# CIS565-Fall-2017/Project3-CUDA-Path-Tracer

Hardware: AMD Instinct MI355X
Metric: Mrays/sec (live paths x bounces) at 800x800 Cornell depth 8 (higher is better)
Workload: dtype f32

## Files before the change

### include/ptmi355.h

```cpp
#ifndef PTMI355_H
#define PTMI355_H

#include <stdint.h>

#ifdef __cplusplus
extern "C" {
#endif

typedef struct pt_vec3 { float x, y, z; } pt_vec3;
typedef struct pt_mat4 { float m[4][4]; } pt_mat4;

enum pt_geom_type { PT_SPHERE = 0, PT_CUBE = 1,
                    PT_TRIANGLE_MESH = 2 };

typedef struct pt_ray { pt_vec3 origin, direction; } pt_ray;

typedef struct pt_geom {
    int32_t type;
    int32_t materialid;
    pt_vec3 translation, rotation, scale;
    pt_mat4 transform, inverseTransform, invTranspose;
} pt_geom;

typedef struct pt_material {
// ... 150 lines not shown
    float   normal_tolerance;
} pt_temporal_params;
int pt_denoise_temporal(const pt_denoise_params *params, const pt_temporal_params *temporal, int iter,
                        float *host_rgb, uint8_t *host_rgba);
int pt_history(float *rgb, float *length);
int pt_history_reset(void);

int pt_set_denoise_albedo(int enable);
int pt_albedo(float *rgb);

typedef struct pt_variance_params { int32_t levels; float sigma_luminance, sigma_normal, sigma_position; } pt_variance_params;
int pt_get_moments(float *m1, float *m2);
int pt_set_moments(const float *m1, const float *m2);
int pt_denoise_variance(const pt_variance_params *params, int iter, float *host_rgb, uint8_t *host_rgba);
int pt_variance(float *host_var);

int pt_denoise_svgf(const pt_variance_params *params, const pt_temporal_params *temporal, int spatial_below, int iter,
                    float *host_rgb, uint8_t *host_rgba);
int pt_svgf_history(float *rgb, float *u1, float *u2, float *length);
int pt_svgf_variance(float *host_var);
int pt_svgf_reset(void);
int pt_get_stats(pt_stats *stats);
long long pt_total_rays(void);
int pt_get_counters(int64_t *rays, int64_t *first_bounce_rays, int64_t *iterations);

enum pt_stage { PT_STAGE_RAYGEN = 0, PT_STAGE_BOUNCE = 1, PT_STAGE_INTERSECT = 2,
                PT_STAGE_SORT = 3, PT_STAGE_GATHER = 4, PT_STAGE_MESH = 5, PT_STAGE_COUNT = 6 };
typedef struct pt_profile {
    double  ms[PT_STAGE_COUNT];
    int64_t launches[PT_STAGE_COUNT];
} pt_profile;
int pt_set_profiling(int enable);
int pt_get_profile(pt_profile *out);
typedef struct pt_bvh_info {
    int32_t nodes, triangles, depth;
    float   pad;
    float   prune;
} pt_bvh_info;
int pt_get_bvh_info(pt_bvh_info *out);
int pt_bvh_build(const pt_triangle *triangles, int count, float *nodes, int node_capacity,
                 int32_t *order, float *grid);
int pt_cull_boxes(const pt_geom *geoms, int count, const float *eye, float *boxes, float *origin_bound, float *reject);
int pt_tri_bounds(const pt_triangle *triangles, int count, float origin_bound, float *bounds);
int pt_tri_records(const pt_triangle *triangles, int count, float origin_bound, uint16_t *records, float frame[4]);
int pt_probe_clock(int microseconds, double *ghz);
int pt_probe_rng(const uint32_t *seeds, int n, int draws, uint32_t *state, float *u);
int pt_probe_sincos(const float *x, uint32_t first_bits, uint32_t n, float *s, float *c, uint64_t sum[2]);
int pt_probe_hemisphere(const float *normals, const uint32_t *seeds, int n, float *dirs);
int pt_probe_sqrt(uint32_t first_bits, uint32_t n, uint64_t mismatch[2]);
int pt_probe_shade_scatter(int iter, int depth, const pt_material *materials, int num_materials, pt_path_segment *paths,
                           const pt_shadeable_intersection *isects, const uint8_t *outside, int n, int deferred);
int pt_probe_glossy_lobe(const float *normals, const uint32_t *seeds, const float *alpha2, int n, float *dirs);
int pt_probe_shade_scatter_glossy(int iter, int depth, const pt_material *materials, int num_materials, pt_path_segment *paths,
                                  const pt_shadeable_intersection *isects, const uint8_t *outside, int n, int deferred);
int pt_probe_environment(const float *texels, int n, const float *dirs, const float *throughput, int count, float *colour);
int pt_probe_texture(const pt_geom *geoms, int num_geoms, const int32_t *hit_geom, const float *points, int count, const float *texels, int n,
                     const float *colour_in, float *colour_out);
int pt_probe_shade_scatter_textured(int iter, int depth, const pt_material *materials, int num_materials, pt_path_segment *paths,
                                    const pt_shadeable_intersection *isects, const uint8_t *outside, int n, int deferred,
                                    const pt_geom *geoms, int num_geoms, const int32_t *hit_geom, const float *tex_texels,
                                    const int32_t *tex_n, const int32_t *tex_offset);
int pt_probe_bump_normal(const pt_geom *geoms, int num_geoms, const int32_t *hit_geom, const float *points, const float *normals, const float *dirs,
                         int count, const float *texels, int n, float *out_normals, uint8_t *perturbed);
int pt_probe_shade_scatter_bumped(int iter, int depth, const pt_material *materials, int num_materials, pt_path_segment *paths,
                                  const pt_shadeable_intersection *isects, const uint8_t *outside, int n, int deferred,
                                  const pt_geom *geoms, int num_geoms, const int32_t *hit_geom, const float *tex_texels,
                                  const int32_t *tex_n, const int32_t *tex_offset, const float *bump_texels, const int32_t *bump_n,
                                  const int32_t *bump_offset);
int pt_probe_smooth_normal(const pt_triangle *triangles, const float *normals, int num_triangles, const int32_t *tri, const float *origins,
                           const float *dirs, int count, float *out_normals, uint8_t *smoothed);
int pt_probe_direct_sample(const pt_geom *geoms, int num_geoms, const pt_material *materials, int num_materials, const float *P,
                           const float *n, const uint32_t *seeds, int count, float *dir, float *weight, int32_t *element);
int pt_probe_shade_scatter_direct(int iter, int depth, int trace_depth, const pt_geom *geoms, int num_geoms, const pt_material *materials,
                                  int num_materials, pt_path_segment *paths, const pt_shadeable_intersection *isects,
                                  const uint8_t *outside, const int32_t *hit_geom, int n);
int pt_probe_sky_sample(const float *texels, int n, const float *normals, const uint32_t *seeds, int count, float *dir, float *weight,
                        int32_t *texel);
int pt_probe_shade_scatter_direct_sky(int iter, int depth, int trace_depth, const pt_geom *geoms, int num_geoms, const pt_material *materials,
                                      int num_materials, pt_path_segment *paths, const pt_shadeable_intersection *isects,
                                      const uint8_t *outside, const int32_t *hit_geom, int n, const float *texels, int env_n);
int pt_probe_tri_form(const pt_triangle *triangles, int count, float origin_bound, const float *origins, const float *directions, int n,
                      uint16_t *ray_slots, int32_t *ray_class, float *form);
int pt_probe_own_surface_plan(uint64_t paths, int ngeoms, int plain_fused);
int pt_num_devices(void);
const char *pt_exchange_transport(void);
const char *pt_last_error(void);
const char *pt_version(void);

#ifdef __cplusplus
}
#endif
#endif
```

### project3-cuda-path-tracer_amd/__init__.py

```python
from .binding import (
    CAMERA_DT, GEOM_DT, ISECT_DT, MATERIAL_DT, MESH_DT, PATH_DT, TRI_DT,
    PT_AA_JITTER, PT_ASYNC_IMAGE, PT_PIN_IMAGE, PT_HOST_SPARSE, PT_SHARED_IMAGE, PT_LOOKAHEAD, PT_GLOSSY, PT_CACHE_FIRST, PT_COMPACT, PT_FAKE_SHADER, PT_MESH_BVH, PT_SORT_MATERIAL, PT_UNFUSED,
    PtError, Scene, Stats, library, pathtrace, pathtraceFree, pathtraceInit,
    device_image_ptr, export_intersections, export_paths, get_image, get_stats, intersect_once,
    set_camera, set_lens, synchronize, tonemap, trace_batch, trace_batch_async, trace_begin, trace_bounce,
    trace_end, clear_image, version, has_experiments, set_profiling, get_profile, STAGES, total_rays, counters, cull_boxes, num_devices, exchange_transport, tri_bounds, tri_records,
    set_image, probe_rng, probe_sincos, probe_sincos_sums, probe_hemisphere, probe_shade_scatter, probe_sqrt, probe_clock, probe_tri_form, probe_own_surface_plan,
    gbuffer, denoise, denoised_device_ptr, DenoiseParams,
    denoise_temporal, history, history_reset, TemporalParams, set_denoise_albedo, albedo,
    set_environment, get_environment, gradient_cubemap, environment_texel, probe_environment,
    glossy_alpha2, probe_glossy_lobe, probe_shade_scatter_glossy,
    PT_DIRECT_LIGHT, LIGHT_DT, light_elements, probe_direct_sample, probe_shade_scatter_direct,
    PT_DIRECT_SKY, sun_on_cubemap, sky_table, probe_sky_sample, probe_shade_scatter_direct_sky,
    PT_TEXTURES, set_texture, get_texture, checker_cubemap, texture_texel, probe_texture, probe_shade_scatter_textured,
    set_bump_map, get_bump_map, studs_bumpmap, bump_normal, probe_bump_normal, probe_shade_scatter_bumped,
    PT_SMOOTH_NORMALS, set_vertex_normals, get_vertex_normals, smooth_normal, probe_smooth_normal,
    PT_MOMENTS, VarianceParams, get_moments, set_moments, denoise_variance, variance,
    denoise_svgf, svgf_history, svgf_variance, svgf_reset,
)
from .build import build
from . import sharding
from . import meshes
from . import host_binding
from .host_binding import build_host, build_ptbench, image_to_rgb8, load_scene, save_pfm, save_png, load_pfm
```

### project3-cuda-path-tracer_amd/binding.py

```python
import ctypes as C
import os

import numpy as np

HERE = os.path.dirname(os.path.abspath(__file__))

GEOM_DT = np.dtype([("type", "<i4"), ("materialid", "<i4"), ("translation", "<f4", 3),
                    ("rotation", "<f4", 3), ("scale", "<f4", 3), ("transform", "<f4", (4, 4)),
                    ("inverseTransform", "<f4", (4, 4)), ("invTranspose", "<f4", (4, 4))])
MATERIAL_DT = np.dtype([("color", "<f4", 3), ("spec_exponent", "<f4"), ("spec_color", "<f4", 3),
                        ("hasReflective", "<f4"), ("hasRefractive", "<f4"),
                        ("indexOfRefraction", "<f4"), ("emittance", "<f4")])
CAMERA_DT = np.dtype([("resolution", "<i4", 2), ("position", "<f4", 3), ("lookAt", "<f4", 3),
                      ("view", "<f4", 3), ("up", "<f4", 3), ("right", "<f4", 3),
                      ("fov", "<f4", 2), ("pixelLength", "<f4", 2)])
PATH_DT = np.dtype([("origin", "<f4", 3), ("direction", "<f4", 3), ("color", "<f4", 3),
                    ("pixelIndex", "<i4"), ("remainingBounces", "<i4")])
ISECT_DT = np.dtype([("t", "<f4"), ("normal", "<f4", 3), ("materialId", "<i4")])
TRI_DT = np.dtype([("v0", "<f4", 3), ("v1", "<f4", 3), ("v2", "<f4", 3)])
MESH_DT = np.dtype([("geom_index", "<i4"), ("first_triangle", "<i4"), ("triangle_count", "<i4")])
LIGHT_DT = np.dtype([("geom", "<i4"), ("kind", "<i4"), ("c0", "<f4", 3), ("ea", "<f4", 3), ("eb", "<f4", 3), ("normal", "<f4", 3),
                     ("area", "<f4"), ("cdf", "<f4"), ("inv_p", "<f4")])

PT_COMPACT, PT_SORT_MATERIAL, PT_FAKE_SHADER, PT_CACHE_FIRST, PT_UNFUSED, PT_MESH_BVH, PT_AA_JITTER, PT_ASYNC_IMAGE, PT_PIN_IMAGE = 1, 2, 4, 8, 16, 32, 64, 128, 256
# ... 101 lines not shown
        L = C.CDLL(path)
        L.pt_last_error.restype = C.c_char_p
        L.pt_version.restype = C.c_char_p
        L.pt_device_image.restype = C.c_void_p
        L.pt_init.argtypes = [C.POINTER(_SceneDesc)]
        L.pt_set_camera.argtypes = [C.c_void_p, C.c_int]
        L.pt_set_lens.argtypes = [C.c_float, C.c_float]
        L.pt_trace.argtypes = [C.c_void_p, C.c_int, C.c_int, C.c_void_p]
        L.pt_trace_batch.argtypes = [C.c_int, C.c_int, C.c_void_p]
        L.pt_trace_batch_async.argtypes = [C.c_int, C.c_int]
        L.pt_trace_begin.argtypes = [C.c_int, C.c_int]
        L.pt_trace_bounce.argtypes = [C.c_int, C.POINTER(C.c_int)]
        L.pt_export_paths.argtypes = [C.c_void_p, C.c_int, C.POINTER(C.c_int)]
        L.pt_export_intersections.argtypes = [C.c_void_p, C.c_void_p, C.c_int]
        L.pt_intersect_once.argtypes = [C.c_void_p, C.c_int, C.c_void_p, C.c_void_p]
        L.pt_get_image.argtypes = [C.c_void_p]
        L.pt_tonemap.argtypes = [C.c_void_p, C.c_int]
        L.pt_get_stats.argtypes = [C.POINTER(Stats)]
        L.pt_total_rays.restype = C.c_int64
        L.pt_get_counters.argtypes = [C.POINTER(C.c_int64)] * 3
        L.pt_set_profiling.argtypes = [C.c_int]
        L.pt_get_profile.argtypes = [C.POINTER(Profile)]
        L.pt_get_bvh_info.argtypes = [C.POINTER(BvhInfo)]
        L.pt_bvh_build.argtypes = [C.c_void_p, C.c_int, C.c_void_p, C.c_int, C.c_void_p, C.c_void_p]
        L.pt_cull_boxes.argtypes = [C.c_void_p, C.c_int, C.c_void_p, C.c_void_p, C.POINTER(C.c_float), C.c_void_p]
        L.pt_tri_bounds.argtypes = [C.c_void_p, C.c_int, C.c_float, C.c_void_p]
        L.pt_tri_records.argtypes = [C.c_void_p, C.c_int, C.c_float, C.c_void_p, C.c_void_p]
        try:
            L.pt_set_image.argtypes = [C.c_void_p]
            L.pt_probe_rng.argtypes = [C.c_void_p, C.c_int, C.c_int, C.c_void_p, C.c_void_p]
            L.pt_probe_sincos.argtypes = [C.c_void_p, C.c_uint32, C.c_uint32, C.c_void_p, C.c_void_p, C.c_void_p]
            L.pt_probe_hemisphere.argtypes = [C.c_void_p, C.c_void_p, C.c_int, C.c_void_p]
            L.pt_probe_sqrt.argtypes = [C.c_uint32, C.c_uint32, C.c_void_p]
            L.pt_probe_shade_scatter.argtypes = [C.c_int, C.c_int, C.c_void_p, C.c_int, C.c_void_p, C.c_void_p, C.c_void_p, C.c_int, C.c_int]
            L.pt_probe_clock.argtypes = [C.c_int, C.POINTER(C.c_double)]
            L.pt_probe_tri_form.argtypes = [C.c_void_p, C.c_int, C.c_float, C.c_void_p, C.c_void_p, C.c_int, C.c_void_p, C.c_void_p, C.c_void_p]
            L.pt_probe_own_surface_plan.argtypes = [C.c_uint64, C.c_int, C.c_int]
            L.pt_gbuffer.argtypes = [C.c_void_p, C.c_void_p, C.c_void_p, C.c_void_p]
            L.pt_denoise.argtypes = [C.POINTER(DenoiseParams), C.c_int, C.c_void_p, C.c_void_p]
            L.pt_denoised_device_image.restype = C.c_void_p
            L.pt_denoise_temporal.argtypes = [C.POINTER(DenoiseParams), C.POINTER(TemporalParams), C.c_int, C.c_void_p, C.c_void_p]
            L.pt_history.argtypes = [C.c_void_p, C.c_void_p]
            L.pt_set_denoise_albedo.argtypes = [C.c_int]
            L.pt_albedo.argtypes = [C.c_void_p]
            L.pt_set_environment.argtypes = [C.c_void_p, C.c_int]
            L.pt_get_environment.argtypes = [C.c_void_p, C.c_int, C.POINTER(C.c_int)]
            L.pt_environment_texel.argtypes = [C.c_void_p, C.c_int, C.c_int, C.c_void_p]
            L.pt_probe_environment.argtypes = [C.c_void_p, C.c_int, C.c_void_p, C.c_void_p, C.c_int, C.c_void_p]
            L.pt_glossy_alpha2.argtypes = [C.c_void_p, C.c_int, C.c_void_p]
            L.pt_probe_glossy_lobe.argtypes = [C.c_void_p, C.c_void_p, C.c_void_p, C.c_int, C.c_void_p]
            L.pt_probe_shade_scatter_glossy.argtypes = L.pt_probe_shade_scatter.argtypes
            L.pt_light_elements.argtypes = [C.c_void_p, C.c_int, C.c_void_p, C.c_int, C.c_void_p, C.c_int]
            L.pt_probe_direct_sample.argtypes = [C.c_void_p, C.c_int, C.c_void_p, C.c_int, C.c_void_p, C.c_void_p, C.c_void_p, C.c_int,
                                                 C.c_void_p, C.c_void_p, C.c_void_p]
            L.pt_probe_shade_scatter_direct.argtypes = [C.c_int, C.c_int, C.c_int, C.c_void_p, C.c_int, C.c_void_p, C.c_int, C.c_void_p,
                                                        C.c_void_p, C.c_void_p, C.c_void_p, C.c_int]
            L.pt_sky_table.argtypes = [C.c_void_p, C.c_int, C.c_void_p, C.c_void_p]
            L.pt_probe_sky_sample.argtypes = [C.c_void_p, C.c_int, C.c_void_p, C.c_void_p, C.c_int, C.c_void_p, C.c_void_p, C.c_void_p]
            L.pt_probe_shade_scatter_direct_sky.argtypes = [C.c_int, C.c_int, C.c_int, C.c_void_p, C.c_int, C.c_void_p, C.c_int, C.c_void_p,
                                                            C.c_void_p, C.c_void_p, C.c_void_p, C.c_int, C.c_void_p, C.c_int]
            L.pt_set_texture.argtypes = [C.c_int, C.c_void_p, C.c_int]
            L.pt_get_texture.argtypes = [C.c_int, C.c_void_p, C.c_int, C.POINTER(C.c_int)]
            L.pt_texture_texel.argtypes = [C.c_void_p, C.c_int, C.c_void_p, C.c_void_p, C.c_int, C.c_int, C.c_void_p]
            L.pt_probe_texture.argtypes = [C.c_void_p, C.c_int, C.c_void_p, C.c_void_p, C.c_int, C.c_void_p, C.c_int, C.c_void_p, C.c_void_p]
            L.pt_probe_shade_scatter_textured.argtypes = L.pt_probe_shade_scatter.argtypes + [C.c_void_p, C.c_int, C.c_void_p, C.c_void_p,
                                                                                              C.c_void_p, C.c_void_p]
            L.pt_set_bump_map.argtypes = L.pt_set_texture.argtypes
            L.pt_get_bump_map.argtypes = L.pt_get_texture.argtypes
            L.pt_bump_normal.argtypes = [C.c_void_p, C.c_int, C.c_void_p, C.c_void_p, C.c_void_p, C.c_void_p, C.c_int, C.c_void_p, C.c_int,
                                         C.c_void_p, C.c_void_p]
            L.pt_probe_bump_normal.argtypes = L.pt_bump_normal.argtypes
            L.pt_probe_shade_scatter_bumped.argtypes = L.pt_probe_shade_scatter_textured.argtypes + [C.c_void_p, C.c_void_p, C.c_void_p]
            L.pt_set_vertex_normals.argtypes = [C.c_void_p, C.c_int]
            L.pt_get_vertex_normals.argtypes = [C.c_void_p, C.c_int, C.POINTER(C.c_int)]
            L.pt_smooth_normal.argtypes = [C.c_void_p, C.c_void_p, C.c_int, C.c_void_p, C.c_void_p, C.c_void_p, C.c_int, C.c_void_p, C.c_void_p]
            L.pt_probe_smooth_normal.argtypes = L.pt_smooth_normal.argtypes
            L.pt_get_moments.argtypes = [C.c_void_p, C.c_void_p]
            L.pt_set_moments.argtypes = [C.c_void_p, C.c_void_p]
            L.pt_denoise_variance.argtypes = [C.POINTER(VarianceParams), C.c_int, C.c_void_p, C.c_void_p]
            L.pt_variance.argtypes = [C.c_void_p]
            L.pt_denoise_svgf.argtypes = [C.POINTER(VarianceParams), C.POINTER(TemporalParams), C.c_int, C.c_int, C.c_void_p, C.c_void_p]
            L.pt_svgf_history.argtypes = [C.c_void_p, C.c_void_p, C.c_void_p, C.c_void_p]
            L.pt_svgf_variance.argtypes = [C.c_void_p]
        except AttributeError:
            if not os.environ.get("PTMI355_LIB"):
                raise
        L.pt_free.restype = None
        L.pt_exchange_transport.restype = C.c_char_p
        _lib = L
    return _lib


def _chk(rc):
    if rc < 0:
        raise PtError("ptmi355 error %d: %s" % (rc, library().pt_last_error().decode()))
    return rc


def _p(a):
    return None if a is None else a.ctypes.data_as(C.c_void_p)


def version():
    return library().pt_version().decode()


def has_experiments():
    return "+experiments" in version()


def pathtraceInit(scene, flags=PT_COMPACT, device=0, stream=None, tile=(0, 1, 8), max_batch=1,
                  device_image=None, lens=(0.0, 0.0), devices=None, pin_image=True, host_sparse=False, vertex_normals=None):
    global _scene, _host_sparse
    if vertex_normals is not None:
        flags |= PT_SMOOTH_NORMALS
    _host_sparse = bool(host_sparse or (flags & PT_HOST_SPARSE))
    d = _SceneDesc()
    d.geoms, d.num_geoms = _p(scene.geoms), len(scene.geoms)
    d.materials, d.num_materials = _p(scene.materials), len(scene.materials)
    d.triangles, d.num_triangles = _p(scene.triangles), 0 if scene.triangles is None else len(scene.triangles)
    d.meshes, d.num_meshes = _p(scene.meshes), 0 if scene.meshes is None else len(scene.meshes)
    C.memmove(C.byref(d.camera), scene.camera.tobytes(), 84)
    d.trace_depth, d.device = scene.traceDepth, device
    d.flags = flags | (PT_PIN_IMAGE if pin_image else 0) | (PT_HOST_SPARSE if host_sparse else 0)
    d.stream = stream
    d.tile_index, d.tile_count, d.strip_rows = tile
    d.max_batch = max_batch
    d.device_image = device_image
    d.lens_radius, d.focal_distance = lens
    devs = None
    if devices is not None:
        devs = np.ascontiguousarray(devices, dtype=np.int32)
        d.devices, d.num_devices = _p(devs), len(devs)
    _chk(library().pt_init(C.byref(d)))
    _scene = scene
    if vertex_normals is not None:
        set_vertex_normals(vertex_normals)


def pathtraceFree():
    global _scene
    library().pt_free()
    _scene = None


def pathtrace(pbo, frame, iteration, copy_image=True):
    if _scene is None:
        raise PtError("pathtrace: pathtraceInit has not been called")
    L = library()
    _chk(L.pt_set_camera(_p(_scene.camera), _scene.traceDepth))
    _chk(L.pt_trace(pbo, frame, iteration, _p(_scene.image) if copy_image else None))
    if _host_sparse:
        view = _scene.image.view()
        view.setflags(write=False)
        return view
    return _scene.image


def set_lens(lens_radius, focal_distance):
    _chk(library().pt_set_lens(lens_radius, focal_distance))


def set_camera(camera, trace_depth):
    cam = np.ascontiguousarray(camera, dtype=CAMERA_DT).reshape(1)
    _chk(library().pt_set_camera(_p(cam), trace_depth))

# ... 587 lines not shown

def tri_bounds(triangles, origin_bound):
    t = np.ascontiguousarray(triangles, dtype=TRI_DT)
    out = np.zeros(((len(t) + 3) & ~3, 4), dtype=np.float32)
    _chk(library().pt_tri_bounds(_p(t), len(t), float(origin_bound), _p(out)))
    return out[:len(t)]


def tri_records(triangles, origin_bound):
    t = np.ascontiguousarray(triangles, dtype=TRI_DT)
    n64 = (len(t) + 63) & ~63
    rec = np.zeros((max(n64, 1), 32), dtype=np.float16)
    frame = np.zeros(4, dtype=np.float32)
    n = _chk(library().pt_tri_records(_p(t), len(t), float(origin_bound), _p(rec), _p(frame)))
    return rec[:n], frame


def total_rays():
    r = library().pt_total_rays()
    if r < 0:
        _chk(int(r))
    return int(r)


def counters():
    a, b, c = C.c_int64(), C.c_int64(), C.c_int64()
    _chk(library().pt_get_counters(C.byref(a), C.byref(b), C.byref(c)))
    return a.value, b.value, c.value


def probe_rng(seeds, draws):
    sd = np.ascontiguousarray(seeds, dtype=np.uint32)
    st = np.zeros(len(sd), dtype=np.uint32)
    u = np.zeros(len(sd), dtype=np.float32)
    _chk(library().pt_probe_rng(_p(sd), len(sd), int(draws), _p(st), _p(u)))
    return st, u


def probe_sincos(x):
    xs = np.ascontiguousarray(x, dtype=np.float32)
    s = np.zeros(len(xs), dtype=np.float32)
    c = np.zeros(len(xs), dtype=np.float32)
    _chk(library().pt_probe_sincos(_p(xs), 0, len(xs), _p(s), _p(c), None))
    return s, c


def probe_sincos_sums(first_bits, count):
    out = np.zeros(2, dtype=np.uint64)
    _chk(library().pt_probe_sincos(None, int(first_bits), int(count), None, None, _p(out)))
    return int(out[0]), int(out[1])


def probe_sqrt(first_bits, count):
    out = np.zeros(2, dtype=np.uint64)
    _chk(library().pt_probe_sqrt(int(first_bits), int(count), _p(out)))
    return int(out[0]), int(out[1])


def probe_clock(microseconds=200):
    ghz = C.c_double(0.0)
    _chk(library().pt_probe_clock(int(microseconds), C.byref(ghz)))
    return float(ghz.value)


def probe_tri_form(triangles, origin_bound, origins, directions):
    t = np.ascontiguousarray(triangles, dtype=TRI_DT)
    o = np.ascontiguousarray(origins, dtype=np.float32).reshape(-1, 3)
    d = np.ascontiguousarray(directions, dtype=np.float32).reshape(-1, 3)
    if len(o) != len(d):
        raise PtError("probe_tri_form: %d origins, %d directions" % (len(o), len(d)))
    n, n64 = len(o), (len(t) + 63) & ~63
    slots = np.zeros((n, 32), dtype=np.float16)
    cls = np.zeros(n, dtype=np.int32)
    form = np.zeros((n, n64), dtype=np.float32)
    got = _chk(library().pt_probe_tri_form(_p(t), len(t), float(origin_bound), _p(o), _p(d), n, _p(slots), _p(cls), _p(form)))
    assert got == n64, (got, n64)
    return slots, cls, form


def probe_own_surface_plan(paths, ngeoms, plain_fused=True):
    return bool(library().pt_probe_own_surface_plan(int(paths), int(ngeoms), 1 if plain_fused else 0))


def probe_hemisphere(normals, seeds):
    nr = np.ascontiguousarray(normals, dtype=np.float32).reshape(-1, 3)
    sd = np.ascontiguousarray(seeds, dtype=np.uint32)
    out = np.zeros((len(sd), 3), dtype=np.float32)
    _chk(library().pt_probe_hemisphere(_p(nr), _p(sd), len(sd), _p(out)))
    return out


def glossy_alpha2(exponents):
    e = np.ascontiguousarray(exponents, dtype=np.float32).reshape(-1)
    out = np.zeros(len(e), dtype=np.float32)
    _chk(library().pt_glossy_alpha2(_p(e), len(e), _p(out)))
    return out


def probe_glossy_lobe(normals, seeds, alpha2):
    nr = np.ascontiguousarray(normals, dtype=np.float32).reshape(-1, 3)
    sd = np.ascontiguousarray(seeds, dtype=np.uint32).reshape(-1)
    a2 = np.ascontiguousarray(np.broadcast_to(np.asarray(alpha2, dtype=np.float32), sd.shape))
    if len(nr) != len(sd):
        raise PtError("probe_glossy_lobe: %d normals, %d seeds" % (len(nr), len(sd)))
    out = np.zeros((len(sd), 3), dtype=np.float32)
    _chk(library().pt_probe_glossy_lobe(_p(nr), _p(sd), _p(a2), len(sd), _p(out)))
    return out


def light_elements(geoms, materials):
    g = np.ascontiguousarray(geoms, dtype=GEOM_DT).reshape(-1)
    m = np.ascontiguousarray(materials, dtype=MATERIAL_DT).reshape(-1)
    L = library()
    need = _chk(L.pt_light_elements(_p(g), len(g), _p(m), len(m), None, 0))
    out = np.zeros(need, dtype=LIGHT_DT)
    if need:
        assert _chk(L.pt_light_elements(_p(g), len(g), _p(m), len(m), _p(out), need)) == need
    return out


def probe_direct_sample(geoms, materials, P, normals, seeds):
    g = np.ascontiguousarray(geoms, dtype=GEOM_DT).reshape(-1)
    m = np.ascontiguousarray(materials, dtype=MATERIAL_DT).reshape(-1)
    p = np.ascontiguousarray(P, dtype=np.float32).reshape(-1, 3)
    nr = np.ascontiguousarray(normals, dtype=np.float32).reshape(-1, 3)
    sd = np.ascontiguousarray(seeds, dtype=np.uint32).reshape(-1)
    if len(p) != len(sd) or len(nr) != len(sd):
        raise PtError("probe_direct_sample: %d points, %d normals, %d seeds" % (len(p), len(nr), len(sd)))
    d = np.zeros((len(sd), 3), dtype=np.float32)
    w = np.zeros(len(sd), dtype=np.float32)
    e = np.zeros(len(sd), dtype=np.int32)
    _chk(library().pt_probe_direct_sample(_p(g), len(g), _p(m), len(m), _p(p), _p(nr), _p(sd), len(sd), _p(d), _p(w), _p(e)))
    return d, w, e


def probe_shade_scatter_direct(iter, depth, trace_depth, geoms, materials, paths, isects, outside=None, hit_geom=None):
    g = np.ascontiguousarray(geoms, dtype=GEOM_DT).reshape(-1)
    m = np.ascontiguousarray(materials, dtype=MATERIAL_DT).reshape(-1)
    p = np.array(paths, dtype=PATH_DT, copy=True, order="C").reshape(-1)
    x = np.ascontiguousarray(isects, dtype=ISECT_DT).reshape(-1)
    o = None if outside is None else np.ascontiguousarray(outside, dtype=np.uint8).reshape(-1)
    h = None if hit_geom is None else np.ascontiguousarray(hit_geom, dtype=np.int32).reshape(-1)
    if len(x) != len(p) or (o is not None and len(o) != len(p)) or (h is not None and len(h) != len(p)):
        raise PtError("probe_shade_scatter_direct: %d paths, %d intersections" % (len(p), len(x)))
    _chk(library().pt_probe_shade_scatter_direct(int(iter), int(depth), int(trace_depth), _p(g), len(g), _p(m), len(m), _p(p), _p(x),
                                                 _p(o), _p(h), len(p)))
    return p


def probe_shade_scatter_glossy(iter, depth, materials, paths, isects, outside=None, deferred=False):
    return probe_shade_scatter(iter, depth, materials, paths, isects, outside, deferred, _glossy=True)


def probe_shade_scatter(iter, depth, materials, paths, isects, outside=None, deferred=False, _glossy=False):
    m = np.ascontiguousarray(materials, dtype=MATERIAL_DT)
    p = np.array(paths, dtype=PATH_DT, copy=True, order="C").reshape(-1)
    x = np.ascontiguousarray(isects, dtype=ISECT_DT).reshape(-1)
    o = None if outside is None else np.ascontiguousarray(outside, dtype=np.uint8).reshape(-1)
    if len(x) != len(p) or (o is not None and len(o) != len(p)):
        raise PtError("probe_shade_scatter: %d paths, %d intersections, %s outside flags" % (len(p), len(x), "no" if o is None else len(o)))
    fn = library().pt_probe_shade_scatter_glossy if _glossy else library().pt_probe_shade_scatter
    _chk(fn(int(iter), int(depth), _p(m), len(m), _p(p), _p(x), _p(o), len(p), 1 if deferred else 0))
    return p
```

### project3-cuda-path-tracer_amd/csrc/pt_h_api.hpp

```cpp
#pragma once

namespace one {

const char *pt_last_error(void) { return g_err; }
const char *pt_version(void) {
#ifdef PT_EXPERIMENTS
    return "ptmi355 0.1 (gfx950, fp32 no-contract, wave64) +experiments";
#else
    return "ptmi355 0.1 (gfx950, fp32 no-contract, wave64)";
#endif
}

void pt_free(void) {
    if (!R.live && !R.scratch) return;
    if (R.stream) (void)hipStreamSynchronize(R.stream);
    for (int k = 0; k < OV_MAX_LANES; ++k) {
        if (R.lane[k].stream) (void)hipStreamSynchronize(R.lane[k].stream);
        if (R.lane[k].la_stream) (void)hipStreamSynchronize(R.lane[k].la_stream);
    }
    if (R.la_gstream) (void)hipStreamSynchronize(R.la_gstream);
    for (int k = 0; k < 2; ++k) if (R.pool_mem[k]) (void)hipFree(R.pool_mem[k]);
    if (R.isect_mem) (void)hipFree(R.isect_mem);
    if (R.sort_table) (void)hipFree(R.sort_table);
    if (R.cache_mem) (void)hipFree(R.cache_mem);
// ... 126 lines not shown
    for (int k = 0; k < d->num_meshes; ++k) {
        const pt_mesh &m = d->meshes[k];
        if (m.geom_index < 0 || m.geom_index >= d->num_geoms || d->geoms[m.geom_index].type != PT_TRIANGLE_MESH ||
            m.first_triangle < 0 || m.triangle_count < 0 ||
            (int64_t)m.first_triangle + (int64_t)m.triangle_count > (int64_t)d->num_triangles)
            return fail(PT_ERR_INVALID, "pt_init: mesh %d is inconsistent", k);
        for (int j = 0; j < k; ++j)
            if (d->meshes[j].geom_index == m.geom_index)
                return fail(PT_ERR_INVALID, "pt_init: geom %d owns more than one mesh", m.geom_index);
    }
    if ((d->flags & PT_CACHE_FIRST) && ((d->flags & PT_AA_JITTER) || d->lens_radius > 0.0f))
        return fail(PT_ERR_INVALID, "pt_init: PT_CACHE_FIRST needs identical camera rays every iteration; it cannot be "
                                    "combined with PT_AA_JITTER or a lens (INSTRUCTION.md:113)");
    if (d->lens_radius > 0.0f && !(d->focal_distance > 0.0f))
        return fail(PT_ERR_INVALID, "pt_init: a lens needs focal_distance > 0");
    std::vector<pt_light_element> light_el;
    if ((d->flags & PT_DIRECT_SKY) && !(d->flags & PT_DIRECT_LIGHT) && !(d->flags & PT_FAKE_SHADER))
        return fail(PT_ERR_INVALID, "pt_init: PT_DIRECT_SKY needs PT_DIRECT_LIGHT (the sky is one more light element of its sampler)");
    if ((d->flags & PT_DIRECT_LIGHT) && !(d->flags & PT_FAKE_SHADER)) {
        if (d->flags & PT_UNFUSED)
            return fail(PT_ERR_INVALID, "pt_init: PT_DIRECT_LIGHT cannot be combined with PT_UNFUSED (its intersection planes do not carry the winning primitive)");
        if (d->flags & PT_CACHE_FIRST)
            return fail(PT_ERR_INVALID, "pt_init: PT_DIRECT_LIGHT cannot be combined with PT_CACHE_FIRST (the table form of bounce 0 has no DIRECT variant)");
        if (d->trace_depth > MAX_DEPTH - 1)
            return fail(PT_ERR_INVALID, "pt_init: PT_DIRECT_LIGHT runs trace_depth + 1 bounces: trace_depth %d outside [1,%d]", d->trace_depth, MAX_DEPTH - 1);
        const int ne = ptlight::elements(d->geoms, d->num_geoms, d->materials, d->num_materials, light_el);
        if (ne < 0) return fail(PT_ERR_INTERNAL, "pt_init: light elements");
        if (ne > ptlight::MAX_ELEMENTS)
            return fail(PT_ERR_INVALID, "pt_init: PT_DIRECT_LIGHT: %d light elements (at most %d)", ne, ptlight::MAX_ELEMENTS);
    }
    if ((d->flags & PT_TEXTURES) && !(d->flags & PT_FAKE_SHADER)) {
        if (d->flags & PT_UNFUSED)
            return fail(PT_ERR_INVALID, "pt_init: PT_TEXTURES cannot be combined with PT_UNFUSED (its intersection planes do not carry the winning primitive)");
        if (d->flags & PT_CACHE_FIRST)
            return fail(PT_ERR_INVALID, "pt_init: PT_TEXTURES cannot be combined with PT_CACHE_FIRST (the table form of bounce 0 has no TEX variant)");
        if (d->flags & PT_DIRECT_LIGHT)
            return fail(PT_ERR_INVALID, "pt_init: PT_TEXTURES cannot be combined with PT_DIRECT_LIGHT (the direct kernels have no textured form yet)");
    }
    if ((d->flags & PT_SMOOTH_NORMALS) && !(d->flags & PT_FAKE_SHADER)) {
        if (d->flags & PT_UNFUSED)
            return fail(PT_ERR_INVALID, "pt_init: PT_SMOOTH_NORMALS cannot be combined with PT_UNFUSED (its intersection planes carry one normal and no triangle)");
        if (d->flags & PT_CACHE_FIRST)
            return fail(PT_ERR_INVALID, "pt_init: PT_SMOOTH_NORMALS cannot be combined with PT_CACHE_FIRST (the table form of bounce 0 has no SMOOTH variant)");
        if (d->flags & PT_TEXTURES)
            return fail(PT_ERR_INVALID, "pt_init: PT_SMOOTH_NORMALS cannot be combined with PT_TEXTURES (the textured kernels have no smooth form yet)");
        if (d->flags & PT_DIRECT_LIGHT)
            return fail(PT_ERR_INVALID, "pt_init: PT_SMOOTH_NORMALS cannot be combined with PT_DIRECT_LIGHT (the direct kernels have no smooth form yet)");
    }
    int ndev = 0;
    if (hipGetDeviceCount(&ndev) != hipSuccess || ndev <= 0)
        return fail(PT_ERR_DEVICE, "pt_init: no HIP device (this library has no CPU fallback)");
    if (d->device < 0 || d->device >= ndev) return fail(PT_ERR_INVALID, "pt_init: device %d of %d", d->device, ndev);
    HIPCHK(hipSetDevice(d->device));

    R = Renderer{};
    R.desc = *d; R.cam = d->camera; R.trace_depth = d->trace_depth; R.flags = d->flags; R.device = d->device;
    R.lens = Lens{(d->flags & PT_AA_JITTER) ? 1 : 0, d->lens_radius, d->focal_distance};
    R.whole_max_paths = 6000000;
    if (const char *wm = getenv("PTMI355_WHOLE_MAX")) R.whole_max_paths = strtoull(wm, nullptr, 10);
    R.whole_max_host_paths = 16000000;
    if (const char *wm = getenv("PTMI355_WHOLE_MAX_HOST")) R.whole_max_host_paths = strtoull(wm, nullptr, 10);
    if (getenv("PTMI355_WHOLE_MAX") && !getenv("PTMI355_WHOLE_MAX_HOST")) R.whole_max_host_paths = R.whole_max_paths;
    if (const char *e = getenv("PTMI355_OVERLAP")) {
        const int nl = atoi(e);
        R.ov_enabled = nl != 0;
        if (nl >= 2) { R.ov_lanes = std::min(nl, OV_MAX_LANES); R.ov_lanes_set = true; }
    }
    if (const char *e = getenv("PTMI355_OVERLAP_GB")) R.ov_budget_gb = atof(e);
    if (const char *e = pt_experiment("PTMI355_LANE_STREAMS")) R.ov_streams = std::max(1, atoi(e));
    R.epi_enabled = true;
    if (const char *e = pt_experiment("PTMI355_HOST_EPILOGUE")) R.epi_enabled = atoi(e) != 0;
    if (d->flags & PT_MOMENTS) R.epi_enabled = false;
    if (const char *e = pt_experiment("PTMI355_EPI_DIRECT")) R.epi_direct_enabled = atoi(e) != 0;
    R.defer_enabled = true;
    if (const char *e = pt_experiment("PTMI355_DEFER_DIR")) R.defer_enabled = atoi(e) != 0;
    R.own_enabled = true;
    if (const char *e = pt_experiment("PTMI355_OWN_SURFACE")) R.own_enabled = atoi(e) != 0;
    R.first_hit_enabled = true;
    if (const char *e = pt_experiment("PTMI355_FIRST_HIT")) R.first_hit_enabled = atoi(e) != 0;
    R.first_two_enabled = true;
    if (const char *e = pt_experiment("PTMI355_FIRST_TWO")) R.first_two_enabled = atoi(e) != 0;
    R.first_state_enabled = true;
    if (const char *e = pt_experiment("PTMI355_FIRST_STATE")) R.first_state_enabled = atoi(e) != 0;
    R.host_sparse_enabled = (d->flags & (PT_HOST_SPARSE | PT_SHARED_IMAGE)) != 0;
    if (const char *e = pt_experiment("PTMI355_ASYNC_DIRECT")) R.async_direct_enabled = atoi(e) != 0;
    R.pin_enabled = true;
    if (const char *e = pt_experiment("PTMI355_PIN")) R.pin_enabled = atoi(e) != 0;
    R.npix = W * H;
    R.map.W = W; R.map.H = H; R.map.tile_index = d->tile_index; R.map.tile_count = tile_count;
    R.map.strip_rows = tile_count > 1 ? d->strip_rows : H;
    R.map.tile_pixels = tile_rows(d->tile_index, tile_count, R.map.strip_rows, H) * W;
    if (R.map.tile_pixels <= 0) return fail(PT_ERR_INVALID, "pt_init: tile owns no rows");
    make_div_magic((uint32_t)R.map.tile_pixels, &R.map.div_magic, &R.map.div_shift);
    auto magic_holds = [](uint32_t d, uint32_t magic, uint32_t shift) {
        auto fast = [&](uint32_t n) {
            if (d == 1) return n;
            const uint32_t q = (uint32_t)(((uint64_t)magic * n) >> 32);
            return (((n - q) >> 1) + q) >> shift;
        };
        for (uint64_t k = 0; k <= 0xffffffffull / d && k < 4096; ++k)
            for (int e = -1; e <= 1; ++e) {
                const uint64_t n = k * d + (uint64_t)(int64_t)e;
                if (n <= 0xffffffffull && fast((uint32_t)n) != (uint32_t)n / d) return false;
            }
        const uint32_t probes[] = {0u, 1u, d - 1, d, d + 1, 0x7fffffffu, 0x80000000u, 0xfffffffeu, 0xffffffffu};
        for (uint32_t n : probes)
            if (fast(n) != n / d) return false;
        return true;
    };
    if (!magic_holds((uint32_t)R.map.tile_pixels, R.map.div_magic, R.map.div_shift))
        return fail(PT_ERR_INTERNAL, "pt_init: division magic failed for n / %d", R.map.tile_pixels);
    if (tile_count > 1) {
        const uint32_t span = (uint32_t)R.map.strip_rows * (uint32_t)W;
        make_div_magic(span, &R.la_tg.magic, &R.la_tg.shift);
        R.la_tg.skip = (uint32_t)(tile_count - 1) * span;
        R.la_tg.first = (uint32_t)d->tile_index * span;
        R.la_tiles_ok = span >= 2 && magic_holds(span, R.la_tg.magic, R.la_tg.shift);
    }
    R.max_batch = d->max_batch < 1 ? 1 : d->max_batch;
    if ((int64_t)R.max_batch * R.map.tile_pixels >= (int64_t)0x3ffffff0)
        return fail(PT_ERR_INVALID, "pt_init: max_batch * tile pixels must stay below 2^30 (32-bit byte offsets into the planes)");
    R.cap = (uint32_t)R.max_batch * (uint32_t)R.map.tile_pixels;
    if (d->stream) { R.stream = (hipStream_t)d->stream; R.own_stream = false; }
    else {
        int lo = 0, hi = 0;
        const char *pe = pt_experiment("PTMI355_MAIN_PRIO");
        if (hipDeviceGetStreamPriorityRange(&lo, &hi) != hipSuccess) { (void)hipGetLastError(); lo = hi = 0; }
        if ((pe && atoi(pe) == 0) || hipStreamCreateWithPriority(&R.stream, hipStreamNonBlocking, hi) != hipSuccess) {
            (void)hipGetLastError();
            HIPCHK(hipStreamCreateWithFlags(&R.stream, hipStreamNonBlocking));
        }
        R.own_stream = true;
    }
    R.live = true;

    std::vector<float> grec((size_t)std::max(1, d->num_geoms) * ptd::GEOM_WORDS, 0.0f);
    for (int i = 0; i < d->num_geoms; ++i) {
        const pt_geom &g = d->geoms[i];
        float *r = grec.data() + (size_t)i * ptd::GEOM_WORDS;
        int first = 0, count = 0, boff = 0;
        for (int k = 0, off = 0; k < d->num_meshes; ++k) {
            if (d->meshes[k].geom_index == i) { first = d->meshes[k].first_triangle; count = d->meshes[k].triangle_count; boff = off; break; }
            off += (d->meshes[k].triangle_count + 63) & ~63;
        }
        memcpy(&r[0], &g.type, 4); memcpy(&r[1], &g.materialid, 4); memcpy(&r[2], &first, 4); memcpy(&r[3], &count, 4);
        const pt_mat4 *ms[3] = {&g.inverseTransform, &g.transform, &g.invTranspose};
        const int offs[3] = {ptd::G_INV, ptd::G_FWD, ptd::G_INVT};
        for (int m = 0; m < 3; ++m)
            for (int c = 0; c < 4; ++c)
                for (int rr = 0; rr < 3; ++rr) r[offs[m] + c * 3 + rr] = ms[m]->m[c][rr];
        if (g.type == PT_TRIANGLE_MESH) memcpy(&r[ptd::G_INV + 6], &boff, 4);
    }
    std::vector<float> mrec((size_t)d->num_materials * ptd::MAT_WORDS, 0.0f);
    pack_materials(d->materials, d->num_materials, mrec.data(), (d->flags & PT_GLOSSY) != 0);
    std::vector<float> trec((size_t)std::max(1, d->num_triangles) * TRI_WORDS, 0.0f);
    for (int i = 0; i < d->num_triangles; ++i) {
        const pt_triangle &t = d->triangles[i];
        float *r = trec.data() + (size_t)i * TRI_WORDS;
        r[0] = t.v0.x; r[1] = t.v0.y; r[2] = t.v0.z;
        r[3] = t.v1.x - t.v0.x; r[4] = t.v1.y - t.v0.y; r[5] = t.v1.z - t.v0.z;
        r[6] = t.v2.x - t.v0.x; r[7] = t.v2.y - t.v0.y; r[8] = t.v2.z - t.v0.z;
    }
    for (int k = 0; k < d->num_meshes; ++k) {
        const pt_mesh &m = d->meshes[k];
        const float pad = ptbvh::spec_pad(reinterpret_cast<const float *>(d->triangles + m.first_triangle), m.triangle_count);
        for (int i = 0; i < m.triangle_count; ++i) trec[(size_t)(m.first_triangle + i) * TRI_WORDS + 10] = pad;
// ... 72 lines not shown
        R.mesh_mode != MESH_BVH && d->num_materials <= 64) {
        bool on = true;
        if (const char *e = pt_experiment("PTMI355_SORT_FUSED")) on = atoi(e) != 0;
        double budget_gb = 96.0;
        if (const char *e = pt_experiment("PTMI355_SORT_FUSED_GB")) budget_gb = atof(e);
        R.sort_runs = 1;
        if (const char *e = pt_experiment("PTMI355_SORT_RUNS")) R.sort_runs = std::max(1, std::min(8, atoi(e)));
        const double tiles_k = (double)d->num_materials * ((double)((R.cap + 63) / 64) + 8192.0 * R.sort_runs);
        if (on && tiles_k * 2560.0 * 2.0 <= budget_gb * 1e9 && tiles_k * 64.0 < 2147483648.0) R.sort_keys = d->num_materials;
    }
    if ((R.flags & PT_DIRECT_LIGHT) && !(R.flags & PT_FAKE_SHADER) && (R.flags & PT_SORT_MATERIAL) && !R.sort_keys)
        return fail(PT_ERR_INVALID, "pt_init: PT_DIRECT_LIGHT cannot be combined with the two-kernel form of PT_SORT_MATERIAL, which this "
                                    "session would take (its intersection planes do not carry the winning primitive)");
    if ((R.flags & PT_TEXTURES) && !(R.flags & PT_FAKE_SHADER) && (R.flags & PT_SORT_MATERIAL) && !R.sort_keys)
        return fail(PT_ERR_INVALID, "pt_init: PT_TEXTURES cannot be combined with the two-kernel form of PT_SORT_MATERIAL, which this "
                                    "session would take (its intersection planes do not carry the winning primitive)");
    if ((R.flags & PT_SMOOTH_NORMALS) && !(R.flags & PT_FAKE_SHADER) && (R.flags & PT_SORT_MATERIAL) && !R.sort_keys)
        return fail(PT_ERR_INVALID, "pt_init: PT_SMOOTH_NORMALS cannot be combined with the two-kernel form of PT_SORT_MATERIAL, which this "
                                    "session would take (its intersection planes carry one normal and no triangle)");
    if (!light_el.empty()) {
        std::vector<float> lrec;
        ptlight::records(d->geoms, light_el, lrec);
        static_assert(ptlight::RECORD_WORDS == ptd::LIGHT_WORDS, "one record layout");
        HIPCHK(hipMalloc((void **)&R.d_lights, lrec.size() * 4));
        HIPCHK(hipMemcpy(R.d_lights, lrec.data(), lrec.size() * 4, hipMemcpyHostToDevice));
        R.nlights = (int)light_el.size();
        if (sky_session()) R.lamp_rec = lrec;
    }
    const size_t capz = R.cap;
    const size_t pool_mult = (size_t)std::max(1, R.sort_keys);
    const size_t run_mult = R.sort_keys > 0 ? (size_t)R.sort_runs : 1;
    for (int k = 0; k < 2; ++k) {
        R.pool_bytes = pool_mult * (((capz + 63) / 64) + 2 * 8192 * run_mult) * 64 * 10 * 4;
        HIPCHK(hipMalloc(&R.pool_mem[k], R.pool_bytes));
        R.pool[k] = carve_pool(R.pool_mem[k], R.cap);
    }
    if ((R.flags & (PT_UNFUSED | PT_FAKE_SHADER)) || ((R.flags & PT_SORT_MATERIAL) && !R.sort_keys)) {
        const int rc = ensure_isect();
        if (rc != PT_OK) return rc;
    }
    R.final_bytes = capz * 4 * 4;
    HIPCHK(hipMalloc(&R.final_mem, R.final_bytes));
    HIPCHK(hipMemsetAsync(R.final_mem, 0, capz * 4 * 4, R.stream));
    R.fin_serial = 0;
    if (const char *e = pt_experiment("PTMI355_FIN_SERIAL")) R.fin_serial = (uint32_t)strtoul(e, nullptr, 0);
    if (d->device_image) { R.image = d->device_image; R.own_image = false; }
    else {
        HIPCHK(hipMalloc(&R.image, (size_t)R.npix * 3 * 4));
        R.own_image = true;
        HIPCHK(hipMemsetAsync(R.image, 0, (size_t)R.npix * 3 * 4, R.stream));
    }
    if (R.flags & PT_MOMENTS) {
        HIPCHK(hipMalloc((void **)&R.mom_mem, (size_t)R.npix * 2 * sizeof(float)));
        HIPCHK(hipMemsetAsync(R.mom_mem, 0, (size_t)R.npix * 2 * sizeof(float), R.stream));
    }
    R.max_tiles = (R.cap + TILE - 1) / TILE;
    R.ctl_bytes = offsetof(Control, bucket) - offsetof(Control, stamp) +
                  (size_t)session_bounces_max(R.trace_depth) * sizeof(((Control *)nullptr)->bucket[0]);
    HIPCHK(hipMalloc((void **)&R.ctl, sizeof(Control)));
    HIPCHK(hipMemsetAsync(R.ctl, 0, sizeof(Control), R.stream));
    HIPCHK(hipMalloc((void **)&R.persist, sizeof(Persist)));
    HIPCHK(hipMemsetAsync(R.persist, 0, sizeof(Persist), R.stream));
    hipDeviceProp_t prop;
    HIPCHK(hipGetDeviceProperties(&prop, d->device));
    const int cus = prop.multiProcessorCount > 0 ? prop.multiProcessorCount : 256;
    int per_cu = 8;
    {
        const bool sorted = R.sort_keys > 0;
        const bool own = R.mesh_mode == MESH_NONE && !sorted;
        auto size_for = [&](auto sh) -> int {
            constexpr int SH = decltype(sh)::value;
            constexpr int SHN = SH & ~SH_SMOOTH;
            const void *fns[2];
            if (R.mesh_mode == MESH_BVH) { fns[0] = bounce_fn<MESH_PRE, SH>(R.scene_lds, false, false); fns[1] = bounce_fn<MESH_PRE, SH>(R.scene_lds, true, false); }
            else if (R.mesh_mode == MESH_TILES) { fns[0] = bounce_fn<MESH_TILES, SH>(R.scene_lds, false, sorted); fns[1] = bounce_fn<MESH_TILES, SH>(R.scene_lds, true, sorted); }
            else { fns[0] = bounce_fn<MESH_NONE, SHN>(R.scene_lds, false, sorted); fns[1] = bounce_fn<MESH_NONE, SHN>(R.scene_lds, true, sorted); }
            const void *fns_own[2] = {own ? bounce_fn<MESH_NONE, SHN>(R.scene_lds, false, false, true) : fns[0], own ? bounce_fn<MESH_NONE, SHN>(R.scene_lds, true, false, true) : fns[1]};
            const void *fns_tab[4] = {own ? bounce_fn<MESH_NONE, SHN>(R.scene_lds, false, false, false, true) : fns[0], own ? bounce_fn<MESH_NONE, SHN>(R.scene_lds, true, false, false, true) : fns[1],
                                      own ? bounce_fn<MESH_NONE, SHN>(R.scene_lds, false, false, true, true) : fns[0], own ? bounce_fn<MESH_NONE, SHN>(R.scene_lds, true, false, true, true) : fns[1]};
            const void *fns_two[2] = {own ? bounce_fn<MESH_NONE, SHN>(R.scene_lds, true, false, false, true, true) : fns[0],
                                      own ? bounce_fn<MESH_NONE, SHN>(R.scene_lds, true, false, true, true, true) : fns[0]};
            const void *fns_state[2] = {own ? bounce_fn<MESH_NONE, SHN>(R.scene_lds, true, false, false, true, true, true) : fns[0],
                                        own ? bounce_fn<MESH_NONE, SHN>(R.scene_lds, true, false, true, true, true, true) : fns[0]};
            for (const void *f : {fns[0], fns[1], fns_own[0], fns_own[1], fns_tab[0], fns_tab[1], fns_tab[2], fns_tab[3], fns_two[0], fns_two[1],
                                  fns_state[0], fns_state[1]}) {
                int n = 0;
                HIPCHK(hipOccupancyMaxActiveBlocksPerMultiprocessor(&n, f, BLOCK, R.lds_bytes));
                per_cu = std::min(per_cu, n);
            }
            return PT_OK;
        };
        int rc = size_for(std::integral_constant<int, 0>{});
        if (rc == PT_OK && (R.nlights > 0 || sky_session())) rc = size_for(std::integral_constant<int, SH_DIRECT>{});
        if (rc == PT_OK && (R.flags & PT_TEXTURES) && !(R.flags & PT_FAKE_SHADER)) rc = size_for(std::integral_constant<int, SH_TEX>{});
        if (rc == PT_OK && (R.flags & PT_SMOOTH_NORMALS) && !(R.flags & PT_FAKE_SHADER) && R.mesh_mode != MESH_NONE)
            rc = size_for(std::integral_constant<int, SH_SMOOTH>{});
        if (rc != PT_OK) return rc;
    }
    if (per_cu < 1) per_cu = 1;
    if (per_cu > 8) per_cu = 8;
    if (const char *e = pt_experiment("PTMI355_WGS_PER_CU")) per_cu = std::max(1, std::min(per_cu, atoi(e)));
    R.grid = (int)std::min<uint32_t>((R.max_tiles + WAVES - 1) / WAVES, (uint32_t)cus * (uint32_t)per_cu);
    R.per_cu = per_cu;
    if (const char *e = pt_experiment("PTMI355_LA_CUS")) R.la_cus = std::max(0, std::min(64, atoi(e) & ~7));
    if (R.grid < 1) R.grid = 1;
    if (R.grid * WAVES > 8192) R.grid = 8192 / WAVES;
    {
        int n = 0;
        HIPCHK(hipOccupancyMaxActiveBlocksPerMultiprocessor(
            &n, R.scene_lds ? (const void *)k_iteration<true> : (const void *)k_iteration<false>, BLOCK, R.lds_bytes));
        n = std::max(1, std::min(n, 8));
        if (const char *e = pt_experiment("PTMI355_WGS_PER_CU")) n = std::max(1, std::min(n, atoi(e)));
        R.grid_iter = (int)std::min<uint32_t>((R.max_tiles + WAVES - 1) / WAVES, (uint32_t)cus * (uint32_t)n);
        R.grid_iter = std::max(1, std::min(R.grid_iter, 8192 / WAVES));
        R.grid_iter_cur = R.grid_iter; R.cus = cus;
        if (const char *e = pt_experiment("PTMI355_ITER_TPW")) R.iter_tpw = std::max(0, atoi(e));
        if (const char *e = pt_experiment("PTMI355_ITER_WGS_ALL")) R.iter_wgs_per_cu_all = std::max(1, atoi(e));
        R.iter_counts_bytes = (size_t)MAX_DEPTH * (size_t)R.grid_iter * 4;
        HIPCHK(hipMalloc((void **)&R.iter_counts, R.iter_counts_bytes));
        void *hs = nullptr, *ds = nullptr;
        if (hipHostMalloc(&hs, sizeof(HostStats), hipHostMallocMapped) == hipSuccess && hipHostGetDevicePointer(&ds, hs, 0) == hipSuccess) {
            memset(hs, 0, sizeof(HostStats));
            R.h_stats = (HostStats *)hs; R.d_stats = (HostStats *)ds;
        } else {
            (void)hipGetLastError();
            if (hs) (void)hipHostFree(hs);
        }
    }
    if (R.mesh_mode == MESH_BVH) {
        R.mesh_hit_bytes = (size_t)(((capz + 63) / 64) * 64) * sizeof(float4);
        HIPCHK(hipMalloc((void **)&R.mesh_hit, R.mesh_hit_bytes));
        R.flag_words = (size_t)R.max_tiles + 2 * (size_t)R.grid * WAVES + 8;
        for (int k = 0; k < 2; ++k) {
            HIPCHK(hipMalloc((void **)&R.mesh_flags[k], R.flag_words * sizeof(unsigned long long)));
            HIPCHK(hipMemsetAsync(R.mesh_flags[k], 0, R.flag_words * sizeof(unsigned long long), R.stream));
        }
        HIPCHK(hipFuncSetAttribute((const void *)k_mesh<true>, hipFuncAttributeMaxDynamicSharedMemorySize, (int)MESH_LDS_BYTES));
        HIPCHK(hipFuncSetAttribute((const void *)k_mesh<false>, hipFuncAttributeMaxDynamicSharedMemorySize, (int)MESH_LDS_BYTES));
        R.grid_mesh = (int)std::min<uint32_t>((R.max_tiles + MESH_WG_WAVES - 1) / MESH_WG_WAVES, (uint32_t)cus);
        if (R.grid_mesh < 1) R.grid_mesh = 1;
    }
    if (R.flags & PT_CACHE_FIRST) {
        HIPCHK(hipMalloc(&R.cache_mem, (size_t)R.map.tile_pixels * Isect::FIRST_HIT_BYTES));
    } else if (R.first_hit_enabled && !(R.flags & (PT_UNFUSED | PT_SORT_MATERIAL | PT_FAKE_SHADER | PT_AA_JITTER)) && R.mesh_mode == MESH_NONE) {
        if (hipMalloc(&R.cache_mem, (size_t)R.map.tile_pixels * Isect::FIRST_HIT_BYTES) != hipSuccess) { (void)hipGetLastError(); R.cache_mem = nullptr; }
        bool fixed0 = R.cache_mem != nullptr && R.first_state_enabled && !(R.flags & PT_GLOSSY);
        for (int m = 0; m < d->num_materials; ++m) fixed0 = fixed0 && !(d->materials[m].hasRefractive > 0.0f);
        if (fixed0) {
            if (hipMalloc(&R.state_mem, first_state_bytes((size_t)R.map.tile_pixels)) != hipSuccess) { (void)hipGetLastError(); R.state_mem = nullptr; }
            if (R.state_mem && R.map.tile_pixels % TILE == 0 &&
                hipMalloc((void **)&R.state_ended, (size_t)(R.map.tile_pixels / TILE) * sizeof(uint32_t)) != hipSuccess) { (void)hipGetLastError(); R.state_ended = nullptr; }
        }
    }
    if ((R.flags & PT_SORT_MATERIAL) && !R.sort_keys) {
        if (d->num_materials + 1 > SORT_MAX_BINS)
            return fail(PT_ERR_INVALID, "pt_init: PT_SORT_MATERIAL keeps one bin per material in LDS: at most %d materials", SORT_MAX_BINS - 1);
        {
            int per_cu_sort = 8;
            if (const char *e = pt_experiment("PTMI355_SORT_WGS")) per_cu_sort = std::max(1, atoi(e));
            R.sort_wave = true;
            if (const char *e = pt_experiment("PTMI355_SORT_WAVE")) R.sort_wave = atoi(e) != 0;
            const uint32_t chunks = (R.cap + SORT_CHUNK - 1) / SORT_CHUNK;
            R.grid_sort = (int)std::max<uint32_t>(1u, std::min<uint32_t>(chunks, (uint32_t)cus * (uint32_t)per_cu_sort));
        }
        HIPCHK(hipMalloc((void **)&R.sort_table, ((size_t)(d->num_materials + 1) * R.grid_sort + 4) * sizeof(uint32_t)));
    }
    {
        const size_t Wp = ((size_t)R.grid * WAVES * pool_mult * run_mult + 3) & ~(size_t)3;
// ... 664 lines not shown
```

### project3-cuda-path-tracer_amd/csrc/pt_h_enqueue.hpp

```cpp
#pragma once

namespace {

BounceArgs bounce_args(int depth) {
    BounceArgs a{};
    a.dbg_counts = R.dbg_counts;
    a.in = R.pool[R.cur];
    a.out = (R.flags & PT_COMPACT) ? R.pool[R.cur ^ 1] : R.pool[R.cur];
    a.isect = R.isect;
    a.scene = R.scene;
    a.map = R.map;
    a.ctl = R.ctl;
    a.dir_in = tile_dir((R.flags & PT_COMPACT) ? R.cur_dir : -1);
    a.dir_out = tile_dir(depth);
    a.fin = R.final_mem;
    a.fin_stamp = R.fin_serial;
    a.cam = R.cam;
    a.lens = R.lens;
    a.depth = depth; a.trace_depth = R.trace_depth; a.iter0 = R.step_iter0;
    a.pool_n = (uint32_t)R.map.tile_pixels * (uint32_t)R.step_count;
    a.gen_rays = (depth == 0 && R.gen_fused) ? 1 : 0;
    a.mesh_hit = R.mesh_hit;
    a.mesh_flags_in = R.mesh_flags[depth & 1]; a.mesh_flags_out = R.mesh_flags[(depth + 1) & 1];
    a.mesh_scan = R.mesh_marked ? 0 : 1;
// ... 37 lines not shown
    R.mesh_marked = false;
    R.self_gathered = false; R.host_stats_serial = 0;
    if (clear) HIPCHK(hipMemsetAsync(&R.ctl->stamp, 0, R.ctl_bytes, R.stream));
    if (R.mesh_mode == MESH_BVH)
        for (int k = 0; k < 2; ++k)
            HIPCHK(hipMemsetAsync(R.mesh_flags[k], 0, R.flag_words * sizeof(unsigned long long), R.stream));
    R.gen_fused = !stepping && (!(R.flags & (PT_UNFUSED | PT_SORT_MATERIAL | PT_FAKE_SHADER)) || R.sort_keys > 0);
    R.gen_sort = !stepping && (R.flags & PT_SORT_MATERIAL) && !R.sort_keys && !(R.flags & PT_FAKE_SHADER) && R.sort_wave &&
                 R.scene.nmats + 1 <= SORTW_MAX_BINS;
    if (R.gen_fused || R.gen_sort) return PT_OK;
    const uint32_t total = (uint32_t)R.map.tile_pixels * (uint32_t)count;
    StageTimer tm(PT_STAGE_RAYGEN);
    hipLaunchKernelGGL(k_raygen, dim3((total + BLOCK - 1) / BLOCK), dim3(BLOCK), 0, R.stream, R.pool[0], R.cam,
                       R.lens, R.map, count, iter0, R.trace_depth, R.ctl);
    HIPCHK(hipGetLastError());
    return PT_OK;
}

#define PT_MESH_DISPATCH(CALL)                                          \
    do {                                                                \
        if (R.scene_lds) {                                              \
            constexpr bool SLDS = true;                                 \
            if (R.mesh_mode == MESH_BVH) { constexpr int MESH = MESH_BVH; CALL; }            \
            else if (R.mesh_mode == MESH_TILES) { constexpr int MESH = MESH_TILES; CALL; }   \
            else { constexpr int MESH = MESH_NONE; CALL; }              \
        } else {                                                        \
            constexpr bool SLDS = false;                                \
            if (R.mesh_mode == MESH_BVH) { constexpr int MESH = MESH_BVH; CALL; }            \
            else if (R.mesh_mode == MESH_TILES) { constexpr int MESH = MESH_TILES; CALL; }   \
            else { constexpr int MESH = MESH_NONE; CALL; }              \
        }                                                               \
    } while (0)

void launch_intersect(const Pool &in, const uint32_t *n_ptr, uint32_t n_fixed, const RangeDir &dir,
                      const uint32_t *nprev, bool raygen_pool = false, bool generate = false) {
    const bool same_rays = !R.lens.aa && !(R.lens.radius > 0.0f);
    const unsigned long long *cull0 = (raygen_pool && R.cull0_tiles && same_rays) ? R.d_cull0 : nullptr;
    RayGen gen{};
    if (generate) {
        gen.cam = R.cam; gen.lens = R.lens; gen.map = R.map; gen.trace_depth = R.trace_depth;
        gen.iter0 = R.step_iter0;
        PT_MESH_DISPATCH(hipLaunchKernelGGL((k_intersect<MESH, SLDS, true>), dim3(R.grid), dim3(BLOCK), R.lds_bytes, R.stream, in,
                                            R.isect, R.scene, n_ptr, n_fixed, dir, nprev, R.ctl, cull0, R.cull0_tiles, gen));
        return;
    }
    PT_MESH_DISPATCH(hipLaunchKernelGGL((k_intersect<MESH, SLDS>), dim3(R.grid), dim3(BLOCK), R.lds_bytes, R.stream, in,
                                        R.isect, R.scene, n_ptr, n_fixed, dir, nprev, R.ctl, cull0, R.cull0_tiles, gen));
}

template <int MESH, int SH = 0>
const void *bounce_fn(bool slds, bool gen, bool sorted, bool own = false, bool table = false, bool first2 = false, bool state2 = false) {
    if constexpr (MESH == MESH_NONE) {
        if (table && !sorted) {
            constexpr int SH0 = SH & (SH_ENV | SH_GLOSSY);
            if (first2 && state2) {
                if (own) return slds ? (const void *)k_bounce<MODE_STATE2, true, MESH, true, true, false, true, 0> : (const void *)k_bounce<MODE_STATE2, true, MESH, false, true, false, true, 0>;
                return slds ? (const void *)k_bounce<MODE_STATE2, true, MESH, true, true, false, false, 0> : (const void *)k_bounce<MODE_STATE2, true, MESH, false, true, false, false, 0>;
            }
            if (first2) {
                if (own) return slds ? (const void *)k_bounce<MODE_FIRST2, true, MESH, true, true, false, true, SH0> : (const void *)k_bounce<MODE_FIRST2, true, MESH, false, true, false, true, SH0>;
                return slds ? (const void *)k_bounce<MODE_FIRST2, true, MESH, true, true, false, false, SH0> : (const void *)k_bounce<MODE_FIRST2, true, MESH, false, true, false, false, SH0>;
            }
            if (own) {
                if (slds) return gen ? (const void *)k_bounce<MODE_CACHE0, true, MESH, true, true, false, true, SH0> : (const void *)k_bounce<MODE_CACHE0, true, MESH, true, false, false, true, SH0>;
                return gen ? (const void *)k_bounce<MODE_CACHE0, true, MESH, false, true, false, true, SH0> : (const void *)k_bounce<MODE_CACHE0, true, MESH, false, false, false, true, SH0>;
            }
            if (slds) return gen ? (const void *)k_bounce<MODE_CACHE0, true, MESH, true, true, false, false, SH0> : (const void *)k_bounce<MODE_CACHE0, true, MESH, true, false, false, false, SH0>;
            return gen ? (const void *)k_bounce<MODE_CACHE0, true, MESH, false, true, false, false, SH0> : (const void *)k_bounce<MODE_CACHE0, true, MESH, false, false, false, false, SH0>;
        }
        if (own && !sorted) {
            if (slds) return gen ? (const void *)k_bounce<MODE_FUSED, true, MESH, true, true, false, true, SH> : (const void *)k_bounce<MODE_FUSED, true, MESH, true, false, false, true, SH>;
            return gen ? (const void *)k_bounce<MODE_FUSED, true, MESH, false, true, false, true, SH> : (const void *)k_bounce<MODE_FUSED, true, MESH, false, false, false, true, SH>;
        }
    }
    if constexpr (MESH != MESH_PRE) {
        if (sorted) {
            if (slds) return gen ? (const void *)k_bounce<MODE_FUSED, true, MESH, true, true, true, false, SH> : (const void *)k_bounce<MODE_FUSED, true, MESH, true, false, true, false, SH>;
            return gen ? (const void *)k_bounce<MODE_FUSED, true, MESH, false, true, true, false, SH> : (const void *)k_bounce<MODE_FUSED, true, MESH, false, false, true, false, SH>;
        }
    }
    if (slds) return gen ? (const void *)k_bounce<MODE_FUSED, true, MESH, true, true, false, false, SH> : (const void *)k_bounce<MODE_FUSED, true, MESH, true, false, false, false, SH>;
    return gen ? (const void *)k_bounce<MODE_FUSED, true, MESH, false, true, false, false, SH> : (const void *)k_bounce<MODE_FUSED, true, MESH, false, false, false, false, SH>;
}
#define PT_SHADE_DISPATCH_WITH(EXTRA, ...)                                                                  \
    do {                                                                                                    \
        switch ((a.env_n ? SH_ENV : 0) | ((R.flags & PT_GLOSSY) ? SH_GLOSSY : 0)) {                         \
        case SH_ENV | SH_GLOSSY: { constexpr int SH = SH_ENV | SH_GLOSSY | (EXTRA); __VA_ARGS__; } break;   \
        case SH_GLOSSY: { constexpr int SH = SH_GLOSSY | (EXTRA); __VA_ARGS__; } break;                     \
        case SH_ENV: { constexpr int SH = SH_ENV | (EXTRA); __VA_ARGS__; } break;                           \
        default: { constexpr int SH = (EXTRA); __VA_ARGS__; } break;                                        \
        }                                                                                                   \
    } while (0)
#define PT_SHADE_DISPATCH(...) PT_SHADE_DISPATCH_WITH(0, __VA_ARGS__)
template <int MODE, bool COMPACT, int MESH, bool SLDS, bool GEN, bool SORT = false, bool OWN = false>
void launch_k_bounce(const BounceArgs &a) {
    if constexpr (MODE == MODE_STATE2) {
        hipLaunchKernelGGL((k_bounce<MODE, COMPACT, MESH, SLDS, GEN, SORT, OWN, 0>), dim3(R.grid), dim3(BLOCK), R.lds_bytes, R.stream, a);
        return;
    } else {
        if constexpr (MODE == MODE_FUSED) {
            if (a.nlights > 0 && a.depth >= a.trace_depth - 1) {
                PT_SHADE_DISPATCH_WITH(SH_DIRECT, hipLaunchKernelGGL((k_bounce<MODE, COMPACT, MESH, SLDS, GEN, SORT, OWN, SH>), dim3(R.grid), dim3(BLOCK), R.lds_bytes, R.stream, a));
                return;
            }
            if (a.tex_tab != nullptr) {
                PT_SHADE_DISPATCH_WITH(SH_TEX, hipLaunchKernelGGL((k_bounce<MODE, COMPACT, MESH, SLDS, GEN, SORT, OWN, SH>), dim3(R.grid), dim3(BLOCK), R.lds_bytes, R.stream, a));
                return;
            }
            if constexpr (MESH != MESH_NONE) {
                if (a.vnormals != nullptr) {
                    PT_SHADE_DISPATCH_WITH(SH_SMOOTH, hipLaunchKernelGGL((k_bounce<MODE, COMPACT, MESH, SLDS, GEN, SORT, OWN, SH>), dim3(R.grid), dim3(BLOCK), R.lds_bytes, R.stream, a));
                    return;
                }
            }
        }
        PT_SHADE_DISPATCH(hipLaunchKernelGGL((k_bounce<MODE, COMPACT, MESH, SLDS, GEN, SORT, OWN, SH>), dim3(R.grid), dim3(BLOCK), R.lds_bytes, R.stream, a));
    }
}
template <int MODE, bool COMPACT, int MESH, bool GEN>
void launch_bounce_at(const BounceArgs &a) {
    if constexpr (MODE == MODE_FUSED && COMPACT && MESH != MESH_PRE) {
        if (R.sort_keys > 0) {
            if (R.scene_lds) launch_k_bounce<MODE, COMPACT, MESH, true, GEN, true>(a);
            else launch_k_bounce<MODE, COMPACT, MESH, false, GEN, true>(a);
            return;
        }
    }
    if constexpr ((MODE == MODE_FUSED || MODE == MODE_CACHE0 || mode_first2(MODE)) && COMPACT && MESH == MESH_NONE) {
        if (R.own_form) {
            if (R.scene_lds) launch_k_bounce<MODE, COMPACT, MESH, true, GEN, false, true>(a);
            else launch_k_bounce<MODE, COMPACT, MESH, false, GEN, false, true>(a);
            return;
        }
    }
    if (R.scene_lds) launch_k_bounce<MODE, COMPACT, MESH, true, GEN>(a);
    else launch_k_bounce<MODE, COMPACT, MESH, false, GEN>(a);
}
template <int MODE, bool COMPACT>
void launch_bounce(const BounceArgs &a) {
    if constexpr (MODE == MODE_ISECT) {
        launch_bounce_at<MODE, COMPACT, MESH_NONE, false>(a);
    } else if constexpr (MODE == MODE_CACHE0) {
        if (a.gen_rays) launch_bounce_at<MODE, COMPACT, MESH_NONE, true>(a); else launch_bounce_at<MODE, COMPACT, MESH_NONE, false>(a);
    } else if constexpr (mode_first2(MODE)) {
        static_assert(COMPACT, "MODE_FIRST2 / MODE_STATE2 compact");
        launch_bounce_at<MODE, COMPACT, MESH_NONE, true>(a);
    } else {
        const bool gen = a.gen_rays != 0;
        if (R.mesh_mode == MESH_BVH) { if (gen) launch_bounce_at<MODE, COMPACT, MESH_PRE, true>(a); else launch_bounce_at<MODE, COMPACT, MESH_PRE, false>(a); }
        else if (R.mesh_mode == MESH_TILES) { if (gen) launch_bounce_at<MODE, COMPACT, MESH_TILES, true>(a); else launch_bounce_at<MODE, COMPACT, MESH_TILES, false>(a); }
        else { if (gen) launch_bounce_at<MODE, COMPACT, MESH_NONE, true>(a); else launch_bounce_at<MODE, COMPACT, MESH_NONE, false>(a); }
    }
}

int enqueue_bounce(int depth, bool may_fuse = false) {
    BounceArgs a = bounce_args(depth);
    R.own_form = false;
    const bool compact = (R.flags & PT_COMPACT) != 0;
    const bool sort2 = (R.flags & PT_SORT_MATERIAL) && R.sort_keys == 0;
    const bool unfused = (R.flags & PT_UNFUSED) != 0 || sort2;
    if (unfused) {
        StageTimer tm(PT_STAGE_INTERSECT);
        const bool generate = depth == 0 && R.gen_sort;
        const uint32_t *n_ptr = (compact && !generate) ? &R.ctl->nlive[depth] : (const uint32_t *)nullptr;
        const uint32_t *nprev = (compact && depth > 0) ? &R.ctl->nlive[depth - 1] : (const uint32_t *)nullptr;
        launch_intersect(a.in, n_ptr, a.pool_n, a.dir_in, nprev, depth == 0, generate);
        HIPCHK(hipGetLastError());
    }
    if (sort2) {
        a.in = R.pool[R.cur]; a.out = R.pool[R.cur ^ 1];
        a.sort_table = R.sort_table; a.nbins = R.scene.nmats + 1;
        a.gen_rays = (depth == 0 && R.gen_sort) ? 1 : 0;
        {
            StageTimer tm(PT_STAGE_SORT);
            const size_t lds = ((size_t)LDS_CTL_WORDS + (size_t)((a.nbins + 3) & ~3)) * 4;
            if (compact) hipLaunchKernelGGL(k_sort_hist<true>, dim3(R.grid_sort), dim3(BLOCK), lds, R.stream, a);
            else hipLaunchKernelGGL(k_sort_hist<false>, dim3(R.grid_sort), dim3(BLOCK), lds, R.stream, a);
            HIPCHK(hipGetLastError());
        }
        StageTimer tm(PT_STAGE_BOUNCE);
        if (a.nbins <= SORTW_MAX_BINS && R.sort_wave) {
            const size_t lds = shade_sorted_w_lds_words(R.scene.nmats) * 4;
#define PT_SORTED_W(COMPACT, GEN) \
    PT_SHADE_DISPATCH(hipLaunchKernelGGL((k_shade_sorted_w<COMPACT, GEN, SH>), dim3(R.grid_sort), dim3(BLOCK), lds, R.stream, a))
            if (a.gen_rays) {
                if (compact) PT_SORTED_W(true, true); else PT_SORTED_W(false, true);
            } else {
                if (compact) PT_SORTED_W(true, false); else PT_SORTED_W(false, false);
            }
#undef PT_SORTED_W
        } else {
            const size_t nb = (size_t)((a.nbins + 3) & ~3);
            const size_t lds = ((size_t)LDS_CTL_WORDS + (3 + WAVES) * nb + 2 * SORT_CHUNK +
                                (a.nbins <= 64 ? (size_t)R.scene.nmats * ptd::MAT_WORDS : 0)) * 4;
            if (compact) PT_SHADE_DISPATCH(hipLaunchKernelGGL((k_shade_sorted<true, SH>), dim3(R.grid_sort), dim3(BLOCK), lds, R.stream, a));
            else PT_SHADE_DISPATCH(hipLaunchKernelGGL((k_shade_sorted<false, SH>), dim3(R.grid_sort), dim3(BLOCK), lds, R.stream, a));
        }
        HIPCHK(hipGetLastError());
        R.cur ^= 1; R.cur_dir = -1;
        R.sorted_isects = true;
        R.step_depth = depth + 1;
        return PT_OK;
    }
    const bool same_rays = !R.lens.aa && !(R.lens.radius > 0.0f);
    const bool auto0 = depth == 0 && !unfused && R.first_hit_enabled && R.cache_mem != nullptr && !(R.flags & PT_FAKE_SHADER) &&
                       R.mesh_mode == MESH_NONE && R.sort_keys == 0 && same_rays && a.tex_tab == nullptr &&
                       !(a.nlights > 0 && depth >= a.trace_depth - 1);
    const bool cached0 = depth == 0 && !unfused && ((R.flags & PT_CACHE_FIRST) || auto0);
    const bool first2 = may_fuse && auto0 && !(R.flags & PT_CACHE_FIRST) && compact && R.gen_fused && R.first_two_enabled &&
                        R.trace_depth >= 2 && !(a.nlights > 0 && 1 >= a.trace_depth - 1);
    const bool state2 = first2 && R.state_mem != nullptr && a.env_n == 0;
    if (first2) {
        depth = 1;
        a.depth = 1;
        a.dir_out = tile_dir(1);
        a.gen_rays = 1;
    }
    a.defer_dir = (compact && !unfused && R.mesh_mode == MESH_NONE && R.sort_keys == 0 && depth + 1 < R.trace_depth &&
                   R.defer_enabled) ? 1 : 0;
    R.own_form = own_surface_plan((uint64_t)a.pool_n, R.scene.ngeoms,
                                  compact && !unfused && R.mesh_mode == MESH_NONE && R.sort_keys == 0 &&
                                  R.own_enabled);
    if (cached0 && !R.cache_valid) {
        StageTimer tm(PT_STAGE_INTERSECT);
        const Isect cache{R.cache_mem, (uint32_t)R.map.tile_pixels};
        const int blocks = std::min(R.grid, (R.map.tile_pixels + BLOCK - 1) / BLOCK);
        const hipStream_t fs = R.lane_cur ? R.lane_main : R.stream;
        PT_MESH_DISPATCH(hipLaunchKernelGGL((k_cache_first<MESH, SLDS>), dim3(blocks), dim3(BLOCK), R.lds_bytes, fs,
                                            cache, R.scene, R.cam, R.map, R.state_mem, R.state_ended));
        HIPCHK(hipGetLastError());
        if (R.lane_cur) {
            HIPCHK(hipEventRecord(R.ov_enter, fs));
            HIPCHK(hipStreamWaitEvent(R.stream, R.ov_enter, 0));
            R.first_hit_refence = true;
        }
        R.cache_valid = true;
        R.first_hit_fills++;
    }
    if (!cached0 && !unfused && R.mesh_mode == MESH_BVH) {
        StageTimer tm(PT_STAGE_MESH);
        if (compact) hipLaunchKernelGGL((k_mesh<true>), dim3(R.grid_mesh), dim3(MESH_BLOCK), MESH_LDS_BYTES, R.stream, a);
        else hipLaunchKernelGGL((k_mesh<false>), dim3(R.grid_mesh), dim3(MESH_BLOCK), MESH_LDS_BYTES, R.stream, a);
        HIPCHK(hipGetLastError());
    }
    StageTimer tm(PT_STAGE_BOUNCE);
    if (cached0) {
        a.isect = Isect{R.cache_mem, (uint32_t)R.map.tile_pixels};
        R.first_hit_launches++;
        if (state2) {
            a.first_state = R.state_mem; a.first_ended = R.state_ended; a.first_ended_tiles = (uint32_t)(R.map.tile_pixels / TILE);
            R.first_two_launches++; R.first_state_launches++; tm.two_bounces(); launch_bounce<MODE_STATE2, true>(a);
        }
        else if (first2) { R.first_two_launches++; tm.two_bounces(); launch_bounce<MODE_FIRST2, true>(a); }
        else if (compact) launch_bounce<MODE_CACHE0, true>(a); else launch_bounce<MODE_CACHE0, false>(a);
    } else if (unfused) {
        if (compact) launch_bounce<MODE_ISECT, true>(a); else launch_bounce<MODE_ISECT, false>(a);
    } else {
        if (compact) launch_bounce<MODE_FUSED, true>(a); else launch_bounce<MODE_FUSED, false>(a);
    }
    HIPCHK(hipGetLastError());
    if (R.mesh_mode == MESH_BVH) {
        R.mesh_marked = !cached0 && !unfused;
    }
    if (compact) { R.cur ^= 1; R.cur_dir = depth; }
    R.pool_own = R.own_form;
    R.step_depth = depth + 1;
    return PT_OK;
}

int enqueue_fake(void) {
    const uint32_t total = (uint32_t)R.map.tile_pixels * (uint32_t)R.step_count;
    launch_intersect(R.pool[R.cur], nullptr, total, tile_dir(-1), nullptr);
    HIPCHK(hipGetLastError());
    hipLaunchKernelGGL(k_shade_fake, dim3((total + BLOCK - 1) / BLOCK), dim3(BLOCK), 0, R.stream, R.pool[R.cur],
                       R.isect, R.scene.mats, R.map, R.step_iter0, total, R.final_mem, R.fin_serial);
    HIPCHK(hipGetLastError());
    R.step_depth = 1;
    return PT_OK;
}

int enqueue_end(void) {
    if (R.self_gathered) { R.whole = false; return PT_OK; }
    if (R.la_tracing) {
        hipLaunchKernelGGL(k_gather<false>, dim3(1), dim3(BLOCK), 0, R.stream, R.image, R.final_mem, R.cap, R.map, R.step_count, R.ctl,
                           R.persist, session_bounces(), 0u, R.whole ? 1 : 0, 1, R.fin_serial, R.iter_counts, (uint32_t)R.grid_iter_cur,
                           (HostStats *)nullptr, Moments{nullptr, nullptr});
        R.whole = false;
        HIPCHK(hipGetLastError());
        HIPCHK(hipEventRecord(R.lane_cur->traced, R.stream));
        R.lane_cur->gathered_valid = false;
        return PT_OK;
    }
    StageTimer tm(PT_STAGE_GATHER);
    hipStream_t gs = R.stream;
    if (R.lane_cur) {
        HIPCHK(hipEventRecord(R.lane_cur->traced, R.stream));
        HIPCHK(hipStreamWaitEvent(R.lane_main, R.lane_cur->traced, 0));
        gs = R.lane_main;
    }
    const auto gather = R.mom_mem ? k_gather<true> : k_gather<false>;
    hipLaunchKernelGGL(gather, dim3((R.map.tile_pixels + BLOCK - 1) / BLOCK), dim3(BLOCK), 0, gs, R.image,
                       R.final_mem, R.cap, R.map,
                       R.step_count, R.ctl, R.persist, (R.flags & PT_FAKE_SHADER) ? 0 : session_bounces(),
                       (R.flags & PT_FAKE_SHADER) ? (uint32_t)R.map.tile_pixels * (uint32_t)R.step_count : 0u,
                       R.whole ? 1 : 0, R.epi_done ? 1 : 0, R.fin_serial, R.iter_counts, (uint32_t)R.grid_iter_cur,
                       (R.whole && R.host_stats_serial) ? R.d_stats : (HostStats *)nullptr,
                       Moments{R.mom_mem, R.mom_mem ? R.mom_mem + R.npix : (float *)nullptr});
    R.whole = false;
    R.image_epoch++;
    HIPCHK(hipGetLastError());
    if (R.lane_cur) {
        HIPCHK(hipEventRecord(R.lane_cur->gathered, gs));
        R.lane_cur->gathered_valid = true;
    }
    return PT_OK;
}

Renderer::Bufs take_bufs(void) {
    Renderer::Bufs b{};
    for (int k = 0; k < 2; ++k) { b.pool_mem[k] = R.pool_mem[k]; b.pool[k] = R.pool[k]; b.mesh_flags[k] = R.mesh_flags[k]; }
    b.final_mem = R.final_mem; b.ctl = R.ctl; b.dir_mem = R.dir_mem; b.mesh_hit = R.mesh_hit; b.iter_counts = R.iter_counts;
    return b;
}
void put_bufs(const Renderer::Bufs &b) {
    for (int k = 0; k < 2; ++k) { R.pool_mem[k] = b.pool_mem[k]; R.pool[k] = b.pool[k]; R.mesh_flags[k] = b.mesh_flags[k]; }
    R.final_mem = b.final_mem; R.ctl = b.ctl; R.dir_mem = b.dir_mem; R.mesh_hit = b.mesh_hit; R.iter_counts = b.iter_counts;
}

void free_lanes(void) {
    for (int k = 0; k < OV_MAX_LANES; ++k) {
        Renderer::Lane &l = R.lane[k];
        if (l.stream && k < R.ov_streams) { (void)hipStreamSynchronize(l.stream); (void)hipStreamDestroy(l.stream); }
        if (l.la_stream && k < R.ov_streams) { (void)hipStreamSynchronize(l.la_stream); (void)hipStreamDestroy(l.la_stream); }
        if (l.traced) (void)hipEventDestroy(l.traced);
        if (l.gathered) (void)hipEventDestroy(l.gathered);
        if (k > 0) {
            for (int j = 0; j < 2; ++j) { if (l.b.pool_mem[j]) (void)hipFree(l.b.pool_mem[j]); if (l.b.mesh_flags[j]) (void)hipFree(l.b.mesh_flags[j]); }
            if (l.b.final_mem) (void)hipFree(l.b.final_mem);
            if (l.b.ctl) (void)hipFree(l.b.ctl);
// ... 210 lines not shown
```

### project3-cuda-path-tracer_amd/csrc/pt_h_scene.hpp

```cpp
#pragma once

namespace {

int upload_tri_bounds(const pt_scene_desc *d, double Rorigin);

int upload_cull(const pt_scene_desc *d, const pt_camera &cam) {
    const int n = d->num_geoms;
    std::vector<const float *> inv((size_t)std::max(1, n));
    std::vector<char> sph((size_t)std::max(1, n)), skip((size_t)std::max(1, n));
    for (int i = 0; i < n; ++i) {
        inv[(size_t)i] = &d->geoms[i].inverseTransform.m[0][0];
        sph[(size_t)i] = d->geoms[i].type == PT_SPHERE;
        skip[(size_t)i] = d->geoms[i].type == PT_TRIANGLE_MESH;
    }
    const double eye[3] = {(double)cam.position.x, (double)cam.position.y, (double)cam.position.z};
    std::vector<ptcull::Box> boxes;
    std::vector<double> pts(eye, eye + 3);
    for (int t = 0; t < d->num_triangles; ++t) {
        const pt_vec3 *v = &d->triangles[t].v0;
        double m = 0.0;
        for (int k = 0; k < 3; ++k) m = std::max(m, (double)std::fabs(v[k].x) + std::fabs(v[k].y) + std::fabs(v[k].z));
        if (t == 0 || m > pts[3]) { if (pts.size() < 6) pts.resize(6, 0.0); pts[3] = m; pts[4] = 0.0; pts[5] = 0.0; }
    }
    R.scene.rmax = ptcull::make_boxes(inv.data(), reinterpret_cast<const bool *>(sph.data()),
                                      reinterpret_cast<const bool *>(skip.data()), n, pts.data(), (int)(pts.size() / 3), boxes);
    std::vector<float> rec((size_t)std::max(1, n) * CULL_WORDS, 0.0f);
    for (int i = 0; i < n; ++i) {
        float *r = rec.data() + (size_t)i * CULL_WORDS;
        for (int k = 0; k < 3; ++k) ptcull::centre_half(boxes[(size_t)i].lo[k], boxes[(size_t)i].hi[k], r[2 * k], r[2 * k + 1]);
        int ax = 3;
        if (d->geoms[i].type == PT_CUBE && !pt_experiment("PTMI355_NO_AXIS_REJECT"))
            ax = ptcull::reject_row(&d->geoms[i].inverseTransform.m[0][0], &r[7]);
        if (ax == 4 && pt_experiment("PTMI355_NO_ROW_REJECT")) ax = 3;
        const int tw = d->geoms[i].type | (ax << 8);
        memcpy(&r[6], &tw, 4);
        const uint32_t ent = ((uint32_t)d->geoms[i].type << 7) | ((uint32_t)i << 9);
        memcpy(&r[11], &ent, 4);
    }
    if (!R.d_cull) HIPCHK(hipMalloc(&R.d_cull, rec.size() * 4));
    HIPCHK(hipMemcpyAsync(R.d_cull, rec.data(), rec.size() * 4, hipMemcpyHostToDevice, R.stream));
    HIPCHK(hipStreamSynchronize(R.stream));
    R.scene.cull = R.d_cull;
    R.cull_eye_reach = std::fabs(eye[0]) + std::fabs(eye[1]) + std::fabs(eye[2]);
    return upload_tri_bounds(d, (double)R.scene.rmax);
}

void make_tri_bounds(const pt_triangle *tris, int count, double Rorigin, float *out) {
    const double u = 0x1p-24;
    const float pad = ptbvh::spec_pad(reinterpret_cast<const float *>(tris), count);
    const int n4 = (count + 3) & ~3;
    for (int i = 0; i < n4; ++i) {
        float *o = out + (size_t)i * 4;
        if (i >= count) { o[0] = o[1] = o[2] = 0.0f; o[3] = -1.0f; continue; }
        const pt_triangle &t = tris[i];
        const float v0[3] = {t.v0.x, t.v0.y, t.v0.z};
        const float e1[3] = {t.v1.x - t.v0.x, t.v1.y - t.v0.y, t.v1.z - t.v0.z};
        const float e2[3] = {t.v2.x - t.v0.x, t.v2.y - t.v0.y, t.v2.z - t.v0.z};
        double c[3], h2 = 0.0, cinf = 0.0;
        bool fin = true;
        for (int a = 0; a < 3; ++a) {
            const float x1 = v0[a] + e1[a], x2 = v0[a] + e2[a];
            const float lo = std::fmin(v0[a], std::fmin(x1, x2)) - pad, hi = std::fmax(v0[a], std::fmax(x1, x2)) + pad;
            if (!std::isfinite(lo) || !std::isfinite(hi)) fin = false;
            c[a] = 0.5 * ((double)lo + (double)hi);
            const double h = 0.5 * ((double)hi - (double)lo);
            h2 += h * h;
            cinf = std::fmax(cinf, std::fabs(c[a]));
        }
        if (!fin || !std::isfinite(Rorigin)) { o[0] = o[1] = o[2] = 0.0f; o[3] = INFINITY; continue; }
        const double R0 = std::sqrt(h2);
        const double reach = Rorigin + cinf + R0;
        const double delta = 2.0 * 1.7320508075688772 * u * reach;
        const double Rs = (R0 + 4.0 * (delta + 0x1p-19 * reach)) * (1.0 + 0x1p-10);
        for (int a = 0; a < 3; ++a) o[a] = (float)c[a];
        o[3] = ptcull::round_up(Rs * Rs);
        if (!std::isfinite(o[3])) o[3] = INFINITY;
    }
}

void make_tri_records(const float *spheres, int n, _Float16 *records, float frame[4]) {
    double lo[3] = {INFINITY, INFINITY, INFINITY}, hi[3] = {-INFINITY, -INFINITY, -INFINITY};
    for (int i = 0; i < n; ++i) {
        const float *sp = spheres + (size_t)i * 4;
        if (!(sp[3] >= 0.0f) || !std::isfinite(sp[3])) continue;
        for (int a = 0; a < 3; ++a) { lo[a] = std::fmin(lo[a], (double)sp[a]); hi[a] = std::fmax(hi[a], (double)sp[a]); }
    }
    double g[3] = {0.0, 0.0, 0.0}, Rm = 0.0;
// ... 211 lines not shown
```

### project3-cuda-path-tracer_amd/csrc/pt_h_session.hpp

```cpp
#pragma once

namespace {

constexpr size_t ERR_BYTES = 512;
char g_err[ERR_BYTES] = "";
thread_local char *t_err = g_err;

int fail(int code, const char *fmt, ...) {
    va_list ap;
    va_start(ap, fmt);
    vsnprintf(t_err, ERR_BYTES, fmt, ap);
    va_end(ap);
    return code;
}

#define HIPCHK(expr)                                                                            \
    do {                                                                                        \
        hipError_t e_ = (expr);                                                                 \
        if (e_ != hipSuccess)                                                                   \
            return fail(PT_ERR_DEVICE, "HIP error (%s:%d): %s: %s", __builtin_strrchr(__FILE__, '/') ? __builtin_strrchr(__FILE__, '/') + 1 : __FILE__, __LINE__, #expr, \
                        hipGetErrorString(e_));                                                 \
    } while (0)

template <class Texel> struct CubeMaps {
    std::vector<std::vector<float>> keep;
    std::vector<int> n;
    Texel *d_texels = nullptr;
    int2 *d_tab = nullptr;
    int count = 0;
};

constexpr int OV_MAX_LANES = 8;
struct Renderer {
    bool live = false;
    pt_scene_desc desc{};
    pt_camera cam{};
    int trace_depth = 0;
    uint32_t flags = 0;
    int device = 0;
    hipStream_t stream = nullptr;
    bool own_stream = false;
    TileMap map{};
    int npix = 0;
    uint32_t cap = 0;
    int max_batch = 1;
    float *pool_mem[2] = {nullptr, nullptr};
    Pool pool[2]{};
    int cur = 0;
    float *isect_mem = nullptr;
    uint32_t *sort_table = nullptr;
    float *cache_mem = nullptr;
    bool cache_valid = false;
    bool first_hit_enabled = true;
    bool first_hit_refence = false;
    bool first_two_enabled = true;
    uint64_t first_two_launches = 0;
    float *state_mem = nullptr;
    uint32_t *state_ended = nullptr;
    bool first_state_enabled = true;
    uint64_t first_state_launches = 0;
    uint64_t first_hit_fills = 0, first_hit_launches = 0;
    Isect isect{};
    float *final_mem = nullptr;
    uint32_t fin_serial = 0;
    float *image = nullptr;
    bool own_image = false;
    float *d_geoms = nullptr, *d_mats = nullptr, *d_tris = nullptr;
    float *d_cull = nullptr, *d_grec = nullptr;
    float *d_tri_bound = nullptr;
    size_t tri_bound_words = 0;
    std::vector<float> grec_frames;
    uint32_t *d_ginfo = nullptr;
    double cull_eye_reach = 0.0;
    std::vector<pt_geom> geoms_keep;
    std::vector<pt_triangle> tris_keep;
    std::vector<pt_mesh> meshes_keep;
    std::vector<float> grec_keep;
    bool scene_lds = true;
    SceneDev scene{};
    float4 *d_env = nullptr;
    int env_n = 0;
    std::vector<float> env_keep;
    float *d_lights = nullptr;
    int nlights = 0;
    std::vector<float> lamp_rec;
    CubeMaps<float4> tex;
    CubeMaps<ptd::bump_texel> bump;
    std::vector<float> vn_keep;
    float *d_vnormals = nullptr;
    size_t lds_bytes = 0;
    Control *ctl = nullptr;
    Persist *persist = nullptr;
    uint32_t *iter_counts = nullptr;
    size_t iter_counts_bytes = 0;
    HostStats *h_stats = nullptr, *d_stats = nullptr;
    bool want_host_stats = false;
    uint32_t host_stats_serial = 0;
    bool self_gathered = false;
    uint32_t *dir_mem = nullptr;
    size_t dir_stride = 0;
    int cur_dir = -1;
    uint32_t max_tiles = 0;
    size_t flag_words = 0;
    size_t ctl_bytes = 0;
    int grid = 0;
    int grid_iter = 0;
    int grid_iter_cur = 0;
    int iter_tpw = 4;
    int iter_wgs_per_cu_all = 15;
    bool ov_lanes_set = false;
    int ov_streams = 2;
    int cus = 0;
    int grid_sort = 0;
    bool sort_wave = true;
    int sort_runs = 1;
    int sort_keys = 0;
    bool sorted_isects = false;
    bool gen_fused = false;
    bool gen_sort = false;
    Lens lens{0, 0.0f, 0.0f};
    uint64_t whole_max_paths = 6000000;
    uint64_t whole_max_host_paths = 16000000;
    bool whole = false;
    struct Bufs {
        float *pool_mem[2]; Pool pool[2]; float *final_mem; Control *ctl; uint32_t *dir_mem;
        float4 *mesh_hit; unsigned long long *mesh_flags[2]; uint32_t *iter_counts;
    };
    struct Lane {
        hipStream_t stream = nullptr;
        Bufs b{};
        hipEvent_t traced = nullptr, gathered = nullptr;
        bool gathered_valid = false;
        hipStream_t la_stream = nullptr;
    } lane[OV_MAX_LANES];
    Lane *lane_cur = nullptr;
    hipStream_t lane_main = nullptr;
    size_t pool_bytes = 0, final_bytes = 0, dir_bytes = 0, mesh_hit_bytes = 0;
    int ov_lanes = 4;
    double ov_budget_gb = 64.0;
    hipEvent_t ov_enter = nullptr;
    bool ov_ready = false;
    bool ov_enabled = true;
    bool ov_ok = false;
// ... 189 lines not shown
```

### project3-cuda-path-tracer_amd/csrc/pt_k_bounce.hpp

```cpp
#pragma once

namespace {

enum { MODE_FUSED = 0, MODE_ISECT = 1, MODE_CACHE0 = 2, MODE_FIRST2 = 3, MODE_STATE2 = 4 };
constexpr bool mode_first2(int mode) { return mode == MODE_FIRST2 || mode == MODE_STATE2; }

template <typename T>
__device__ __forceinline__ T karg_field(size_t offset) {
    const __attribute__((address_space(4))) char *kp = (const __attribute__((address_space(4))) char *)__builtin_amdgcn_kernarg_segment_ptr();
    asm volatile("" : "+s"(kp));
    return *(const __attribute__((address_space(4))) T *)(kp + offset);
}
template <typename T>
__device__ __forceinline__ T karg_struct(size_t offset) {
    static_assert(sizeof(T) % 4 == 0, "whole dwords");
    const __attribute__((address_space(4))) char *kp = (const __attribute__((address_space(4))) char *)__builtin_amdgcn_kernarg_segment_ptr();
    asm volatile("" : "+s"(kp));
    uint32_t w[sizeof(T) / 4];
#pragma unroll
    for (size_t k = 0; k < sizeof(T) / 4; ++k) w[k] = *(const __attribute__((address_space(4))) uint32_t *)(kp + offset + 4 * k);
    T t;
    __builtin_memcpy(&t, w, sizeof(T));
    return t;
}
__device__ __forceinline__ Pool karg_pool(size_t offset) {
    return Pool{karg_field<float *>(offset + offsetof(Pool, base)), karg_field<uint32_t>(offset + offsetof(Pool, cap))};
}

struct TileCtx {
    bool kargs = false;
    bool kmisc = false;
    bool epi_direct = false;
    SceneAcc acc;
    float *tri_lds;
    int lane, iter0;
    uint32_t stamp;
};

struct TileRegs {
    bool have, active;
    bool miss0;
    uint32_t i, src, tile, pid, smp;
    int pixel;
    f3 col;
    MeshBest mb;
};

template <bool GEN, bool RESOLVE = false, bool OWN = false>
__device__ __forceinline__ void tile_load(const BounceArgs &a, const TileCtx &c, const Pool &in, int depth,
                                          uint32_t tile, uint32_t i, uint32_t src, bool have, bool active,
                                          TileRegs &tr, f3 &ro, f3 &rd, uint32_t &own) {
    own = 0u;
    constexpr bool gen_rays = GEN;
    tr.have = have; tr.i = i; tr.src = src; tr.tile = tile;
    tr.miss0 = false;
    tr.pid = DEAD_PID; tr.smp = 0; tr.pixel = 0;
    tr.col = ptd::mk(1.0f, 1.0f, 1.0f);
    tr.mb.t = FLT_MAX; tr.mb.geom = -1; tr.mb.tri = -1;
    ro = ptd::mk(0, 0, 0); rd = ptd::mk(0, 0, 1);
    if (active) {
        if (gen_rays) {
            tr.pid = i;
        } else {
            const SlotPtr p = (c.kargs ? karg_pool(offsetof(BounceArgs, in)) : in).slot(src);
            tr.pid = ppid(p);
            ro = ptd::mk(pf(p, 0), pf(p, 1), pf(p, 2));
            rd = ptd::mk(pf(p, 3), pf(p, 4), pf(p, 5));
            tr.col = ptd::mk(pf(p, 6), pf(p, 7), pf(p, 8));
            if (tr.pid == DEAD_PID) active = false;
        }
    }
    bool pending = false;
    if (RESOLVE && active) { pending = (tr.pid & PENDING_DIR) != 0u; tr.pid &= ~PENDING_DIR; }
    if (OWN && !GEN && active) { own = (tr.pid & OWN_MASK) >> OWN_SHIFT; tr.pid &= ~OWN_MASK; }
    if (active) {
        if (c.kmisc) {
            const TileMap map = karg_struct<TileMap>(offsetof(BounceArgs, map));
            tr.smp = sample_of(map, tr.pid);
            tr.pixel = local_to_pixel(map, (int)(tr.pid - tr.smp * (uint32_t)map.tile_pixels));
            if (gen_rays) camera_ray(karg_struct<pt_camera>(offsetof(BounceArgs, cam)), karg_struct<Lens>(offsetof(BounceArgs, lens)),
                                     karg_field<int>(offsetof(BounceArgs, trace_depth)), c.iter0 + (int)tr.smp, tr.pixel, map.W, ro, rd);
        } else {
            tr.smp = sample_of(a.map, tr.pid);
            tr.pixel = local_to_pixel(a.map, (int)(tr.pid - tr.smp * (uint32_t)a.map.tile_pixels));
            if (gen_rays) camera_ray(a.cam, a.lens, a.trace_depth, c.iter0 + (int)tr.smp, tr.pixel, a.map.W, ro, rd);
        }
    }
    if (RESOLVE && pending) {
        uint32_t rng = ptd::seeded_engine(c.iter0 + (int)tr.smp, tr.pixel, depth - 1);
        rd = ptd::hemisphere(rd, rng);
    }
    tr.active = active;
}

template <bool OWN, int SH>
__device__ __forceinline__ void tile_first(const BounceArgs &a, const TileCtx &c, TileRegs &tr, f3 &ro, f3 &rd, uint32_t &own) {
    constexpr bool ENV = (SH & SH_ENV) != 0, GLOSSY = (SH & SH_GLOSSY) != 0;
    bool alive = false;
    if (tr.active) {
        const Isect tab = c.kargs ? karg_struct<Isect>(offsetof(BounceArgs, isect)) : a.isect;
        const uint32_t tile_pixels = (uint32_t)(c.kargs ? karg_field<int>(offsetof(BounceArgs, map) + offsetof(TileMap, tile_pixels)) : a.map.tile_pixels);
        const size_t k = tr.pid - tr.smp * tile_pixels;
        const float4 h = *tab.first_hit(k);
        const int2 id = *tab.first_id(k);
        bool deferred = false, missed = false;
        ptd::PathState ps;
        ps.o = ro; ps.d = rd; ps.c = tr.col;
        alive = ptd::shade_scatter<GLOSSY>(ps, h.x, ptd::mk(h.y, h.z, h.w), id.x & 0x7fffffff, (id.x < 0) ? 0 : 1, c.acc.mats,
                                           c.iter0 + (int)tr.smp, tr.pixel, 0, false, false, &deferred, ENV ? &missed : nullptr);
        if (alive) {
            ro = ps.o; rd = ps.d; tr.col = ps.c;
            if (OWN) own = (uint32_t)(id.y + 1);
        } else if (ENV && missed) {
            tr.miss0 = true;
        } else {
            put_final(c.kargs ? karg_field<float *>(offsetof(BounceArgs, fin)) : a.fin, tr.pid, ps.c, c.stamp);
        }
    }
    tr.active = alive;
}

template <bool OWN>
__device__ __forceinline__ void tile_state(const BounceArgs &a, const TileCtx &c, uint32_t tile, uint32_t i, bool have, bool active,
                                           TileRegs &tr, f3 &ro, f3 &rd, uint32_t &own) {
    own = 0u;
    tr.have = have; tr.i = i; tr.src = i; tr.tile = tile;
    tr.miss0 = false;
    tr.pid = DEAD_PID; tr.smp = 0; tr.pixel = 0;
    tr.col = ptd::mk(1.0f, 1.0f, 1.0f);
    tr.mb.t = FLT_MAX; tr.mb.geom = -1; tr.mb.tri = -1;
    ro = ptd::mk(0, 0, 0); rd = ptd::mk(0, 0, 1);
    bool alive = false;
    if (active) {
        tr.pid = i;
        tr.smp = sample_of(a.map, tr.pid);
        const uint32_t k = tr.pid - tr.smp * (uint32_t)a.map.tile_pixels;
        tr.pixel = local_to_pixel(a.map, (int)k);
        const SlotPtr p = Pool{karg_field<float *>(offsetof(BounceArgs, first_state)), 0u}.slot(k);
        const uint32_t word = ppid(p);
        const f3 so = ptd::mk(pf(p, 0), pf(p, 1), pf(p, 2));
        const f3 sd = ptd::mk(pf(p, 3), pf(p, 4), pf(p, 5));
        const f3 sc = ptd::mk(pf(p, 6), pf(p, 7), pf(p, 8));
        const uint32_t kind = word & FS_KIND_MASK;
        if (kind == FS_DIFFUSE || kind == FS_FIXED) {
            alive = true;
            ro = so; rd = sd; tr.col = sc;
            if (OWN) own = (word & OWN_MASK) >> OWN_SHIFT;
// ... 206 lines not shown
        bool have, active;
        uint32_t i, src;
        if (own_span) {
            const uint32_t L = tile * TILE + lane;
            have = true; active = L < ws.total;
            uint32_t off = L, b = ws.b0;
            if (L >= ws.p1) { off = L - ws.p1; b = ws.b1; }
            if (L >= ws.p2) { off = L - ws.p2; b = ws.b2; }
            if (L >= ws.p3) { off = L - ws.p3; b = ws.b3; }
            src = b + off; i = src;
        } else if (aligned) {
            have = tile < tiles;
            active = false; i = 0; src = 0;
            if (have) {
                const uint32_t *tb = a.dir_in.tbase();
                while (tile >= tb[cur + 1]) ++cur;
                const uint32_t t64 = (tile - tb[cur]) * TILE + (uint32_t)lane;
                active = t64 < a.dir_in.count()[cur];
                src = cur * span_in + t64;
                i = a.dir_in.base()[cur] + t64;
            }
        } else {
            have = tile < tiles;
            i = tile * TILE + lane;
            active = have && i < n;
            src = i;
            if (packed_in && have) src = resolve_src(a.dir_in, span_in, cur, i, active, a.ctl);
        }
        TileRegs tr;
        f3 ro, rd;
        uint32_t own;
        if constexpr (MODE == MODE_STATE2) {
            tile_state<OWN>(a, c, tile, i, have, active, tr, ro, rd, own);
            if (ballot64(tr.active) == 0) continue;
        } else {
            tile_load<GEN, RESOLVE, OWN>(a, c, in, depth, tile, i, src, have, active, tr, ro, rd, own);
        }
        if (MODE == MODE_FIRST2) tile_first<OWN, SH>(a, c, tr, ro, rd, own);
        if (MODE == MODE_FUSED || mode_first2(MODE)) {
            const float4 *pre_hit = nullptr;
            if (MESH == MESH_PRE && tr.active) {
                unsigned long long *fl = c.kargs ? karg_field<unsigned long long *>(offsetof(BounceArgs, mesh_flags_in)) : a.mesh_flags_in;
                const unsigned long long word = fl[src >> 6];
                if ((word >> (src & 63u)) & 1ull) pre_hit = (c.kargs ? karg_field<float4 *>(offsetof(BounceArgs, mesh_hit)) : a.mesh_hit) + src;
                if (word != 0ull && (uint32_t)lane == (uint32_t)__builtin_ctzll((unsigned long long)ballot64(tr.active))) fl[src >> 6] = 0ull;
            }
            cull_scene<MESH, OWN>(a.scene, c.acc, q, par, c.tri_lds, tr.active, ro, rd, tr.mb, pre_hit, masked, gmask,
                                  (OWN && (!GEN || mode_first2(MODE))) ? own_surface_miss(c.acc, own, ro, rd) : 0xffffffffu);
            const uint32_t ticket = q.total;
            if (pending) {
                drain_to(q, c.acc, prev_ticket);
                tile_finish<COMPACT, MESH, SORT, DEFER, OWN, SH, MODE == MODE_FIRST2>(a, c, q, par ^ 1, in, out, depth, prev, n, dst_base, packed, traced, key_stride);
            }
            prev = tr; prev_ticket = ticket; pending = true; par ^= 1;
        } else if (MODE == MODE_CACHE0) {
            float t = -1.0f; f3 nrm = ptd::mk(0, 0, 0); int mat = 0, outside = 1, geom = -1;
            if (tr.active) {
                const size_t k = tr.pid - tr.smp * (uint32_t)a.map.tile_pixels;
                const float4 h = *a.isect.first_hit(k);
                const int2 id = *a.isect.first_id(k);
                t = h.x; nrm = ptd::mk(h.y, h.z, h.w);
                mat = id.x & 0x7fffffff; outside = (id.x < 0) ? 0 : 1; geom = id.y;
            }
            tile_shade<COMPACT, MESH_NONE, false, DEFER, SH>(a, c, in, out, depth, tr, ro, rd, t, nrm, mat, outside, n, dst_base, packed, traced, 0,
                                                             OWN ? (uint32_t)(geom + 1) << OWN_SHIFT : 0u, geom);
        } else {
            float t = -1.0f; f3 nrm = ptd::mk(0, 0, 0); int mat = 0, outside = 1;
            if (tr.active) {
                const uint32_t k = i;
                t = at(a.isect.plane(0), k);
                nrm = ptd::mk(at(a.isect.plane(1), k), at(a.isect.plane(2), k), at(a.isect.plane(3), k));
                const int m = at(a.isect.mat(), k);
                mat = m & 0x7fffffff; outside = (m < 0) ? 0 : 1;
            }
            tile_shade<COMPACT, MESH_NONE, false, DEFER, SH>(a, c, in, out, depth, tr, ro, rd, t, nrm, mat, outside, n, dst_base, packed, traced);
        }
    }
    if (pending) {
        drain_to(q, c.acc, prev_ticket);
        tile_finish<COMPACT, MESH, SORT, DEFER, OWN, SH, MODE == MODE_FIRST2>(a, c, q, par ^ 1, in, out, depth, prev, n, dst_base, packed, traced, key_stride);
    }
}

#ifdef PT_WAVE_TIMES
__device__ unsigned long long g_wave_times[8][8192][2];
__device__ uint32_t g_wave_hw[8][8192];
#endif

template <int MODE, bool COMPACT, int MESH, bool SLDS, bool GEN = false, bool SORT = false, bool OWN = false, int SH = 0>
__global__ __launch_bounds__(BLOCK, MESH == MESH_TILES ? PT_LOOP_WAVES : (MESH == MESH_PRE && PT_PRE_WAVES > PT_MIN_WAVES) ? PT_PRE_WAVES : (SORT && MODE == MODE_FUSED && MESH == MESH_NONE) ? PT_SORT_WAVES : ((MODE == MODE_FUSED || MODE == MODE_CACHE0 || mode_first2(MODE)) && COMPACT && MESH == MESH_NONE && !SORT && PT_FUSED_WAVES > PT_MIN_WAVES) ? PT_FUSED_WAVES : PT_MIN_WAVES) void k_bounce(BounceArgs a) {
    static_assert(!OWN || ((MODE == MODE_FUSED || MODE == MODE_CACHE0 || mode_first2(MODE)) && COMPACT && MESH == MESH_NONE && !SORT),
                  "own-surface form: the plain fused compacting kernel, or the table form of its bounce 0");
    static_assert(!mode_first2(MODE) || (COMPACT && MESH == MESH_NONE && GEN && !SORT), "MODE_FIRST2 / MODE_STATE2: the plain compacting pipeline's first launch");
    static_assert(MODE != MODE_STATE2 || SH == 0, "MODE_STATE2: sessions without environment map or lobes");
    static_assert((SH & SH_SMOOTH) == 0 || (MODE == MODE_FUSED && MESH != MESH_NONE), "the SMOOTH forms: the fused kernel of a session with a mesh");
#ifdef PT_WAVE_TIMES
    const unsigned long long wt0 = __builtin_amdgcn_s_memrealtime();
#endif
    extern __shared__ __attribute__((aligned(16))) float lds_raw[];
    uint32_t *sctl = reinterpret_cast<uint32_t *>(lds_raw);
    const LdsCarve lc = carve_lds(lds_raw, a.scene, SLDS);
    TileCtx c;
#ifndef PT_NO_KARG_RELOAD
    c.kargs = MESH != MESH_TILES;
#endif
    c.tri_lds = lc.tri;
#ifdef PT_STAMPS
#define STAMP(k) do { if (blockIdx.x == 0 && threadIdx.x == 0 && a.depth == PT_STAMPS) a.ctl->stamp[k] = __builtin_amdgcn_s_memrealtime(); } while (0)
#else
#define STAMP(k) do {} while (0)
#endif
    STAMP(0);
    c.acc = stage_scene<SLDS>(lc.scene, a.scene);
    STAMP(1);
    WaveQ q{lc.pw, 0, 0};
    const int lane = threadIdx.x & 63;
    c.lane = lane;
    const uint32_t Wp = gridDim.x * WAVES;
    constexpr bool DEFER = COMPACT && MESH == MESH_NONE && !SORT && MODE != MODE_ISECT;
    constexpr bool RESOLVE = MODE == MODE_FUSED && COMPACT && MESH == MESH_NONE && !SORT && !GEN;
    const uint32_t W = (SORT && COMPACT) ? a.dir_out.W : Wp;
    const uint32_t runs_per_wave = (SORT && COMPACT) ? W / Wp : 1u;
    const uint32_t wid0 = run_id();
    c.iter0 = a.iter0;
    c.stamp = a.fin_stamp;
    const uint32_t n = (COMPACT && !GEN) ? a.ctl->nlive[a.depth] : a.pool_n;
    const bool packed_in = COMPACT && !GEN && a.dir_in.mem != nullptr;
    constexpr bool ALIGNED = PT_ALIGNED_TILES && MODE == MODE_FUSED && COMPACT && !GEN && !SORT;
    const bool aligned = ALIGNED && packed_in;
    const uint32_t tiles = aligned ? a.dir_in.tbase()[a.dir_in.nr] : (n + TILE - 1) / TILE;
    const uint32_t R = (tiles + W - 1) / W;
    const uint32_t span_in = packed_in ? *a.dir_in.span() : 0;
    uint32_t traced = 0;
    if (GEN && blockIdx.x == 0 && threadIdx.x == 0) a.ctl->nlive[0] = a.pool_n;
    for (uint32_t j = 0; j < runs_per_wave; ++j) {
        const uint32_t wid = j * Wp + wid0;
        uint32_t packed = 0;
        uint32_t cur = 0;
        if (packed_in && wid * R < tiles)
            cur = aligned ? find_range(a.dir_in.tbase(), a.dir_in.nr, wid * R) : find_range(a.dir_in.base(), a.dir_in.nr, wid * R * TILE);
        STAMP(2);
        run_tiles<MODE, COMPACT, MESH, GEN, SORT, DEFER, RESOLVE, OWN, SH>(a, c, q, a.in, a.out, a.depth, wid * R, R, tiles, n, packed_in, span_in,
                                                  cur, wid * R * TILE, false, WgSpans{}, packed, traced, W * R * TILE, aligned);
        if (COMPACT) {
            if (SORT) {
                if ((uint32_t)lane * W < a.dir_out.nr)
                    __hip_atomic_store(&a.dir_out.count()[(uint32_t)lane * W + wid], packed, __ATOMIC_RELAXED, __HIP_MEMORY_SCOPE_AGENT);
            } else if (lane == 0)
                __hip_atomic_store(&a.dir_out.count()[wid], packed, __ATOMIC_RELAXED, __HIP_MEMORY_SCOPE_AGENT);
        }
    }
    const uint32_t wid = wid0;
    STAMP(6);
#ifdef PT_WAVE_TIMES
    if (lane == 0 && a.depth < 8 && wid < 8192) {
        g_wave_times[a.depth][wid][0] = wt0; g_wave_times[a.depth][wid][1] = __builtin_amdgcn_s_memrealtime();
        uint32_t xcc, hwid;
        asm volatile("s_getreg_b32 %0, hwreg(HW_REG_XCC_ID)" : "=s"(xcc));
        asm volatile("s_getreg_b32 %0, hwreg(HW_REG_HW_ID)" : "=s"(hwid));
        g_wave_hw[a.depth][wid] = (xcc & 0xf) | (hwid << 4);
    }
#endif
    if (mode_first2(MODE)) {
        if (blockIdx.x == 0 && threadIdx.x == 0) a.ctl->alive[0] = n;
        if (lane == 0) sctl[8 + (threadIdx.x >> 6)] = traced;
        __syncthreads();
        if (threadIdx.x == 0) {
            const uint32_t tb = sctl[8] + sctl[9] + sctl[10] + sctl[11];
            if (tb) { atomicAdd(&a.ctl->nlive[1], tb); atomicAdd(&a.ctl->alive[1], tb); }
        }
    } else if (COMPACT) {
        if (blockIdx.x == 0 && threadIdx.x == 0) a.ctl->alive[a.depth] = n;
    } else {
        if (lane == 0) sctl[8 + (threadIdx.x >> 6)] = traced;
        __syncthreads();
        if (threadIdx.x == 0) {
            const uint32_t tb = sctl[8] + sctl[9] + sctl[10] + sctl[11];
            if (tb) atomicAdd(&a.ctl->alive[a.depth], tb);
        }
    }

    if (COMPACT) {
        asm volatile("s_waitcnt vmcnt(0)" ::: "memory");
        __syncthreads();
        if (threadIdx.x == 0) {
            const bool last = elect_last(a.ctl->bucket[a.depth][0], &a.ctl->done[a.depth]);
            if (last) {
                __builtin_amdgcn_fence(__ATOMIC_ACQUIRE, "agent");
                asm volatile("s_waitcnt vmcnt(0)" ::: "memory");
            }
            sctl[0] = last ? 1u : 0u;
        }
        __syncthreads();
        STAMP(7);
        if (sctl[0]) {
            const unsigned long long t0 = __builtin_amdgcn_s_memrealtime();
            scan_range_counts(a.dir_out, &a.ctl->nlive[a.depth + 1], sctl + 16, R * TILE, PT_ALIGNED_TILES && !SORT);
            if (threadIdx.x == 0) a.ctl->scan_ticks[a.depth] = (uint32_t)(__builtin_amdgcn_s_memrealtime() - t0);
#ifdef PT_STAMPS
            if (threadIdx.x == 0 && a.depth == PT_STAMPS) { a.ctl->stamp[8] = t0; a.ctl->stamp[9] = __builtin_amdgcn_s_memrealtime(); }
#endif
        }
    }
}

__device__ __forceinline__ void fold_iter_counts(const uint32_t *counts, uint32_t G, int depth, Control *ctl, Persist *per, HostStats *hs,
                                                 uint32_t iterations, uint32_t serial, uint32_t *lds ) {
    constexpr int PER_PASS = BLOCK / 32;
    unsigned long long rays = 0;
    uint32_t first = 0;
    for (int d0 = 0; d0 < depth; d0 += PER_PASS) {
        const int d = d0 + (int)(threadIdx.x >> 5);
        uint32_t sum = 0;
        if (d < depth)
            for (uint32_t b = threadIdx.x & 31u; b < G; b += 32u)
                sum += __hip_atomic_load(&counts[(uint32_t)d * G + b], __ATOMIC_RELAXED, __HIP_MEMORY_SCOPE_AGENT);
        for (int off = 16; off > 0; off >>= 1) sum += __shfl_down(sum, off, 32);
        if ((threadIdx.x & 31u) == 0) lds[threadIdx.x >> 5] = sum;
        __syncthreads();
        if (threadIdx.x == 0)
            for (int k = 0; k < PER_PASS && d0 + k < depth; ++k) {
                const uint32_t tot = lds[k];
                ctl->alive[d0 + k] = tot;
                if (hs) hs->alive[d0 + k] = tot;
// ... 138 lines not shown
```

### project3-cuda-path-tracer_amd/csrc/pt_probe.hpp

```cpp
#pragma once

namespace {

__global__ void k_probe_rng(const uint32_t *seeds, int n, int draws, uint32_t *state, float *u) {
    const int i = blockIdx.x * blockDim.x + threadIdx.x;
    if (i >= n) return;
    uint32_t st = ptd::lcg_seed(seeds[i]);
    float last = 0.0f;
    for (int k = 0; k < draws; ++k) last = ptd::u01(st);
    if (state) state[i] = st;
    if (u) u[i] = last;
}

__global__ void k_probe_sincos(const float *x, uint32_t first_bits, uint32_t n, float *s, float *c, unsigned long long *sum) {
    unsigned long long as = 0, ac = 0;
    for (uint64_t k = (uint64_t)blockIdx.x * blockDim.x + threadIdx.x; k < n; k += (uint64_t)gridDim.x * blockDim.x) {
        const float v = x ? x[k] : __uint_as_float(first_bits + (uint32_t)k);
        float sv, cv;
        ptd::sincos_shared(v, sv, cv);
        if (s) s[k] = sv;
        if (c) c[k] = cv;
        as += (unsigned long long)__float_as_uint(sv) * (2ull * k + 1ull);
        ac += (unsigned long long)__float_as_uint(cv) * (2ull * k + 1ull);
    }
// ... 450 lines not shown

int pt_probe_rng(const uint32_t *seeds, int n, int draws, uint32_t *state, float *u) {
    if (n < 0 || draws < 0 || (n > 0 && !seeds)) return fail(PT_ERR_INVALID, "pt_probe_rng: bad argument");
    if (n == 0) return PT_OK;
    ProbeBufs b;
    const uint32_t *d_seeds = b.in(seeds, (size_t)n);
    uint32_t *d_state = b.out<uint32_t>((size_t)n);
    float *d_u = b.out<float>((size_t)n);
    if (!b.ok()) return probe_no_device("pt_probe_rng");
    hipLaunchKernelGGL(k_probe_rng, dim3((unsigned)((n + 255) / 256)), dim3(256), 0, 0, d_seeds, n, draws, d_state, d_u);
    HIPCHK(hipGetLastError());
    HIPCHK(b.fetch(state, d_state, (size_t)n));
    HIPCHK(b.fetch(u, d_u, (size_t)n));
    HIPCHK(hipDeviceSynchronize());
    return PT_OK;
}

int pt_probe_sincos(const float *x, uint32_t first_bits, uint32_t n, float *s, float *c, uint64_t sum[2]) {
    if (n == 0) { if (sum) sum[0] = sum[1] = 0; return PT_OK; }
    if ((x || s || c) && n > (1u << 28)) return fail(PT_ERR_INVALID, "pt_probe_sincos: %u elements with arrays (at most 2^28)", n);
    ProbeBufs b;
    const float *d_x = b.in(x, (size_t)n);
    float *d_s = s ? b.out<float>((size_t)n) : nullptr;
    float *d_c = c ? b.out<float>((size_t)n) : nullptr;
    unsigned long long *d_sum = b.out<unsigned long long>(2);
    if (!b.ok()) return probe_no_device("pt_probe_sincos");
    const unsigned blocks = (unsigned)std::min<uint64_t>(((uint64_t)n + 255) / 256, 4096);
    hipLaunchKernelGGL(k_probe_sincos, dim3(blocks), dim3(256), 0, 0, d_x, first_bits, n, d_s, d_c, d_sum);
    HIPCHK(hipGetLastError());
    HIPCHK(b.fetch(s, d_s, (size_t)n));
    HIPCHK(b.fetch(c, d_c, (size_t)n));
    HIPCHK(b.fetch((unsigned long long *)sum, d_sum, 2));
    HIPCHK(hipDeviceSynchronize());
    return PT_OK;
}

int pt_probe_sqrt(uint32_t first_bits, uint32_t n, uint64_t mismatch[2]) {
    if (!mismatch) return fail(PT_ERR_INVALID, "pt_probe_sqrt: null result");
    mismatch[0] = mismatch[1] = 0;
    if (n == 0) return PT_OK;
    ProbeBufs b;
    unsigned long long *d_bad = b.out<unsigned long long>(2);
    if (!b.ok()) return probe_no_device("pt_probe_sqrt");
    const unsigned blocks = (unsigned)std::min<uint64_t>(((uint64_t)n + 255) / 256, 8192);
    hipLaunchKernelGGL(k_probe_sqrt, dim3(blocks), dim3(256), 0, 0, first_bits, n, d_bad);
    HIPCHK(hipGetLastError());
    HIPCHK(b.fetch((unsigned long long *)mismatch, d_bad, 2));
    HIPCHK(hipDeviceSynchronize());
    return PT_OK;
}

int pt_probe_clock(int microseconds, double *ghz) {
    if (!ghz || microseconds < 1 || microseconds > 100000) return fail(PT_ERR_INVALID, "pt_probe_clock: bad argument");
    *ghz = 0.0;
    unsigned long long *h = nullptr, *d = nullptr;
    hipStream_t st = nullptr;
    int lo = 0, hi = 0;
    if (hipHostMalloc((void **)&h, 16, hipHostMallocMapped) != hipSuccess || hipHostGetDevicePointer((void **)&d, h, 0) != hipSuccess) {
        (void)hipGetLastError();
        if (h) (void)hipHostFree(h);
        return fail(PT_ERR_DEVICE, "pt_probe_clock: no HIP device / no mappable host memory (this library has no CPU fallback)");
    }
    h[0] = h[1] = 0;
    if (hipDeviceGetStreamPriorityRange(&lo, &hi) != hipSuccess) { (void)hipGetLastError(); lo = hi = 0; }
    hipError_t e = hipStreamCreateWithPriority(&st, hipStreamNonBlocking, hi);
    if (e == hipSuccess) {
        hipLaunchKernelGGL(k_probe_clock, dim3(1), dim3(64), 0, st, d, (unsigned)microseconds * 100u);
        e = hipGetLastError();
        if (e == hipSuccess) e = hipStreamSynchronize(st);
        (void)hipStreamDestroy(st);
    }
    const unsigned long long cycles = h[0], ticks = h[1];
    (void)hipHostFree(h);
    if (e != hipSuccess) return fail(PT_ERR_DEVICE, "pt_probe_clock: %s", hipGetErrorString(e));
    if (!ticks) return fail(PT_ERR_INTERNAL, "pt_probe_clock: the probe left no counts");
    *ghz = (double)cycles / ((double)ticks * 10.0);
    return PT_OK;
}

int pt_probe_own_surface_plan(uint64_t paths, int ngeoms, int plain_fused) {
    return own_surface_plan(paths, ngeoms, plain_fused != 0) ? 1 : 0;
}

int pt_probe_hemisphere(const float *normals, const uint32_t *seeds, int n, float *dirs) {
    if (n < 0 || (n > 0 && (!normals || !seeds || !dirs))) return fail(PT_ERR_INVALID, "pt_probe_hemisphere: bad argument");
    if (n == 0) return PT_OK;
    ProbeBufs b;
    const float *d_n = b.in(normals, 3 * (size_t)n);
    const uint32_t *d_seeds = b.in(seeds, (size_t)n);
    float *d_d = b.out<float>(3 * (size_t)n);
    if (!b.ok()) return probe_no_device("pt_probe_hemisphere");
    hipLaunchKernelGGL(k_probe_hemisphere, dim3((unsigned)((n + 255) / 256)), dim3(256), 0, 0, d_n, d_seeds, n, d_d);
    HIPCHK(hipGetLastError());
    HIPCHK(b.fetch(dirs, d_d, 3 * (size_t)n));
    HIPCHK(hipDeviceSynchronize());
    return PT_OK;
}

int pt_glossy_alpha2(const float *exponents, int count, float *alpha2) {
    if (count < 0 || (count > 0 && (!exponents || !alpha2))) return fail(PT_ERR_INVALID, "pt_glossy_alpha2: bad argument (count %d)", count);
    for (int i = 0; i < count; ++i) alpha2[i] = one::glossy_alpha2(exponents[i]);
    return PT_OK;
}

int pt_probe_glossy_lobe(const float *normals, const uint32_t *seeds, const float *alpha2, int n, float *dirs) {
    if (n < 0 || (n > 0 && (!normals || !seeds || !alpha2 || !dirs))) return fail(PT_ERR_INVALID, "pt_probe_glossy_lobe: bad argument");
    if (n == 0) return PT_OK;
    ProbeBufs b;
    const float *d_n = b.in(normals, 3 * (size_t)n);
    const uint32_t *d_seeds = b.in(seeds, (size_t)n);
    const float *d_a = b.in(alpha2, (size_t)n);
    float *d_d = b.out<float>(3 * (size_t)n);
    if (!b.ok()) return probe_no_device("pt_probe_glossy_lobe");
    hipLaunchKernelGGL(k_probe_glossy_lobe, dim3((unsigned)((n + 255) / 256)), dim3(256), 0, 0, d_n, d_seeds, d_a, n, d_d);
    HIPCHK(hipGetLastError());
    HIPCHK(b.fetch(dirs, d_d, 3 * (size_t)n));
    HIPCHK(hipDeviceSynchronize());
    return PT_OK;
}

int pt_probe_shade_scatter(int iter, int depth, const pt_material *materials, int num_materials, pt_path_segment *paths,
                           const pt_shadeable_intersection *isects, const uint8_t *outside, int n, int deferred) {
    return probe_shade_scatter("pt_probe_shade_scatter", false, iter, depth, materials, num_materials, paths, isects, outside, n, deferred);
}

int pt_probe_shade_scatter_glossy(int iter, int depth, const pt_material *materials, int num_materials, pt_path_segment *paths,
                                  const pt_shadeable_intersection *isects, const uint8_t *outside, int n, int deferred) {
    return probe_shade_scatter("pt_probe_shade_scatter_glossy", true, iter, depth, materials, num_materials, paths, isects, outside, n,
                               deferred);
}

int pt_probe_direct_sample(const pt_geom *geoms, int num_geoms, const pt_material *materials, int num_materials, const float *P,
                           const float *n, const uint32_t *seeds, int count, float *dir, float *weight, int32_t *element) {
    if (count < 0 || count > (1 << 26) || (count > 0 && (!P || !n || !seeds || !dir || !weight || !element)))
        return fail(PT_ERR_INVALID, "pt_probe_direct_sample: bad argument");
    std::vector<float> rec;
    const int ne = probe_light_records("pt_probe_direct_sample", geoms, num_geoms, materials, num_materials, rec);
    if (ne < 0) return ne;
    if (count == 0) return PT_OK;
    if (ne == 0) {
        for (int i = 0; i < count; ++i) { dir[3 * i] = dir[3 * i + 1] = dir[3 * i + 2] = 0.0f; weight[i] = 0.0f; element[i] = -1; }
        return PT_OK;
    }
    ProbeBufs b;
    const float *d_l = b.in(rec.data(), rec.size());
    const float *d_p = b.in(P, 3 * (size_t)count);
    const float *d_n = b.in(n, 3 * (size_t)count);
    const uint32_t *d_s = b.in(seeds, (size_t)count);
    float *d_d = b.out<float>(3 * (size_t)count);
    float *d_w = b.out<float>((size_t)count);
    int32_t *d_e = b.out<int32_t>((size_t)count);
    if (!b.ok()) return probe_no_device("pt_probe_direct_sample");
    hipLaunchKernelGGL(k_probe_direct_sample, dim3((unsigned)((count + 63) / 64)), dim3(64), 0, 0, d_l, ne, d_p, d_n, d_s, count, d_d, d_w, d_e);
    HIPCHK(hipGetLastError());
    HIPCHK(b.fetch(dir, d_d, 3 * (size_t)count));
    HIPCHK(b.fetch(weight, d_w, (size_t)count));
    HIPCHK(b.fetch(element, d_e, (size_t)count));
    HIPCHK(hipDeviceSynchronize());
    return PT_OK;
}

int pt_probe_shade_scatter_direct(int iter, int depth, int trace_depth, const pt_geom *geoms, int num_geoms, const pt_material *materials,
                                  int num_materials, pt_path_segment *paths, const pt_shadeable_intersection *isects,
                                  const uint8_t *outside, const int32_t *hit_geom, int n) {
    return probe_shade_scatter_direct("pt_probe_shade_scatter_direct", iter, depth, trace_depth, geoms, num_geoms, materials, num_materials,
                                      paths, isects, outside, hit_geom, n, nullptr, 0);
// ... 322 lines not shown
```

### project3-cuda-path-tracer_amd/csrc/pt_types.hpp

```cpp
#pragma once

namespace {


#ifndef PT_MIN_WAVES
#define PT_MIN_WAVES 4
#endif
#ifndef PT_FUSED_WAVES
#define PT_FUSED_WAVES 6
#endif
#ifndef PT_ISECT_WAVES
#define PT_ISECT_WAVES 4
#endif
#ifndef PT_PRE_WAVES
#define PT_PRE_WAVES 6
#endif
#ifndef PT_ITER_WAVES
#define PT_ITER_WAVES PT_MIN_WAVES
#endif
#ifndef PT_SORT_WAVES
#define PT_SORT_WAVES 6
#endif
#ifndef PT_LOOP_WAVES
#define PT_LOOP_WAVES 3
#endif
constexpr int BLOCK = 256;
constexpr int WAVES = BLOCK / 64;
constexpr int TILE = 64;
constexpr int TRI_WORDS = 12;
constexpr int BVH_NODE_WORDS = 16;
enum { MESH_NONE = 0, MESH_TILES = 1, MESH_BVH = 2, MESH_PRE = 3 };
constexpr int MAX_DEPTH = 64;
constexpr uint32_t DEAD_PID = 0xffffffffu;
constexpr uint32_t PENDING_DIR = 0x80000000u;
constexpr int OWN_SHIFT = 26;
constexpr uint32_t OWN_MASK = 0xfu << OWN_SHIFT;
constexpr int OWN_MAX_GEOMS = 15;
constexpr uint64_t OWN_MAX_PATHS = 1ull << OWN_SHIFT;
inline bool own_surface_plan(uint64_t paths, int ngeoms, bool plain_fused) {
    return plain_fused && ngeoms >= 1 && ngeoms <= OWN_MAX_GEOMS && paths <= OWN_MAX_PATHS;
}

template <typename T>
__device__ __forceinline__ T &at(T *plane, uint32_t i) {
    return *reinterpret_cast<T *>(reinterpret_cast<char *>(plane) + (i << 2));
}

#ifndef PT_POOL_QUADS
#define PT_POOL_QUADS 1
#endif
#if PT_POOL_QUADS
struct SlotPtr { char *q, *c; };
struct Pool {
    float *base;
    uint32_t cap;
    __device__ __forceinline__ SlotPtr slot(uint32_t s) const {
        char *t = reinterpret_cast<char *>(base) + (size_t)(s >> 6) * 2560u;
        return SlotPtr{t + ((s & 63u) << 4), t + 2048u + ((s & 63u) << 3)};
    }
    __device__ __forceinline__ float &f(uint32_t s, int k) const {
        const SlotPtr p = slot(s);
        return *reinterpret_cast<float *>(k < 8 ? p.q + (k >> 2) * 1024 + (k & 3) * 4 : p.c);
    }
    __device__ __forceinline__ uint32_t &pid(uint32_t s) const { return *reinterpret_cast<uint32_t *>(slot(s).c + 4); }
};
__device__ __forceinline__ float &pf(const SlotPtr &p, int k) { return *reinterpret_cast<float *>(k < 8 ? p.q + (k >> 2) * 1024 + (k & 3) * 4 : p.c); }
__device__ __forceinline__ uint32_t &ppid(const SlotPtr &p) { return *reinterpret_cast<uint32_t *>(p.c + 4); }
#else
typedef char *SlotPtr;
struct Pool {
    float *base;
    uint32_t cap;
    __device__ __forceinline__ char *slot(uint32_t s) const {
        return reinterpret_cast<char *>(base) + (size_t)(s >> 6) * 2560u + ((s & 63u) << 3);
    }
    __device__ __forceinline__ float &f(uint32_t s, int k) const { return *reinterpret_cast<float *>(slot(s) + (k >> 1) * 512 + (k & 1) * 4); }
    __device__ __forceinline__ uint32_t &pid(uint32_t s) const { return *reinterpret_cast<uint32_t *>(slot(s) + 4 * 512 + 4); }
};
__device__ __forceinline__ float &pf(char *slot, int k) { return *reinterpret_cast<float *>(slot + (k >> 1) * 512 + (k & 1) * 4); }
__device__ __forceinline__ uint32_t &ppid(char *slot) { return *reinterpret_cast<uint32_t *>(slot + 4 * 512 + 4); }
#endif

struct Isect {
    float *base;
    uint32_t cap;
    __device__ __forceinline__ float *plane(int k) const { return base + (size_t)k * cap; }
    __device__ __forceinline__ int *mat() const { return reinterpret_cast<int *>(base + (size_t)4 * cap); }
    __device__ __forceinline__ float4 *first_hit(size_t k) const { return reinterpret_cast<float4 *>(base) + k; }
    __device__ __forceinline__ int2 *first_id(size_t k) const { return reinterpret_cast<int2 *>(base + (size_t)4 * cap) + k; }
    static constexpr size_t FIRST_HIT_BYTES = 24;
};

struct TileMap {
    int W, H;
    int tile_index, tile_count, strip_rows;
    int tile_pixels;
    uint32_t div_magic;
    uint32_t div_shift;
};

__device__ __forceinline__ uint32_t sample_of(const TileMap &m, uint32_t pid) {
    if (m.tile_pixels == 1) return pid;
    const uint32_t q = __umulhi(m.div_magic, pid);
    return (((pid - q) >> 1) + q) >> m.div_shift;
}

struct TileGather {
    uint32_t magic, shift, skip, first;
};

struct Control {
    uint32_t keep[16];
    unsigned long long stamp[16];
    uint32_t nlive[MAX_DEPTH + 1];
    uint32_t alive[MAX_DEPTH + 1];
    uint32_t done[MAX_DEPTH];
    uint32_t done_sort[MAX_DEPTH];
    uint32_t error;
    uint32_t scan_ticks[MAX_DEPTH];
    uint32_t pad[512 - 16 - 32 - 2 * (MAX_DEPTH + 1) - 3 * MAX_DEPTH - 1];
    uint32_t bucket[MAX_DEPTH][2][32 * 16];
    uint32_t ticket[33 * 16];
};
// ... 44 lines not shown
    return __builtin_amdgcn_readfirstlane((threadIdx.x >> 6) * gridDim.x + blockIdx.x);
}

__host__ __device__ __forceinline__ uint32_t range_tiles(uint32_t n, uint32_t W) {
    const uint32_t tiles = (n + 63u) / 64u;
    return (tiles + W - 1) / W;
}

struct Persist {
    unsigned long long rays;
    unsigned long long iterations;
    unsigned long long first_rays;
};

struct HostStats {
    uint32_t alive[MAX_DEPTH + 1];
    uint32_t error;
    uint32_t serial;
};

struct Lens {
    int aa;
    float radius, focal;
};

struct SceneDev {
    const float *geoms;  int ngeoms;
    const float *cull;
    const float *grec;
    const uint32_t *ginfo;
    float rmax;
    const float *mats;   int nmats;
    const float *tris;   int ntris;
    const void *tri_rec;
    const float *bvh_nodes;
    const float *bvh_tris;
    float bvh_prune;  int bvh_guard;
    const int4 *bvh_meshes; int bvh_nmesh;
    const float *bvh_top;  int bvh_top_n;
};

struct BounceArgs {
    unsigned int *dbg_counts;
    Pool in, out;
    Lens lens;
    Isect isect;
    SceneDev scene;
    TileMap map;
    Control *ctl;
    RangeDir dir_in;
    RangeDir dir_out;
    float *fin;
    uint32_t fin_stamp;
    pt_camera cam;
    int depth, trace_depth, iter0;
    uint32_t pool_n;
    int gen_rays;
    float4 *mesh_hit;
    unsigned long long *mesh_flags_in, *mesh_flags_out;
    int mesh_scan;
    const unsigned long long *cam_mask;
    const unsigned long long *cull0;
    uint32_t cull0_tiles;
    float *epi_image, *epi_host;
    int epi_direct;
    uint32_t *iter_counts;
    Persist *persist;
    HostStats *host_stats;
    uint32_t *sort_table;
    int nbins;
    int defer_dir;
    const float4 *env;
    int env_n;
    const float *lights;
    int nlights;
    const float4 *tex;
    const int2 *tex_tab;
    const ptd::bump_texel *bumps;
    const int2 *bump_tab;
    float *first_state;
    const uint32_t *first_ended;
    uint32_t first_ended_tiles;
    const float *vnormals;
};

enum : uint32_t { FS_ZERO = 0, FS_CONST = 1, FS_DIFFUSE = 2, FS_FIXED = 3, FS_KIND_MASK = 3 };
__host__ __device__ constexpr size_t first_state_bytes(size_t tile_pixels) { return ((tile_pixels + 63) / 64) * 2560; }

enum : int {
    SH_ENV = 1,
    SH_GLOSSY = 2,
    SH_DIRECT = 4,
    SH_TEX = 8,
    SH_SMOOTH = 16
};

struct RayGen {
    pt_camera cam;
    Lens lens;
    TileMap map;
    int trace_depth, iter0;
};

__device__ __forceinline__ int local_to_pixel(const TileMap &m, int j) {
    if (m.tile_count == 1) return j;
    int ly = j / m.W;
    int x = j - ly * m.W;
    int ls = ly / m.strip_rows;
    int y = (ls * m.tile_count + m.tile_index) * m.strip_rows + (ly - ls * m.strip_rows);
    return x + y * m.W;
}

__device__ __forceinline__ void camera_ray(const pt_camera &cam, const Lens &lens, int trace_depth, int iter,
                                           int pix, int W, f3 &ro, f3 &rd) {
    const int y = pix / W;
    const int x = pix - y * W;
    f3 view = ptd::mk(cam.view.x, cam.view.y, cam.view.z);
    f3 right = ptd::mk(cam.right.x, cam.right.y, cam.right.z);
    f3 up = ptd::mk(cam.up.x, cam.up.y, cam.up.z);
    f3 pos = ptd::mk(cam.position.x, cam.position.y, cam.position.z);
    float fx = (float)x, fy = (float)y;
    uint32_t rng = 0;
    if (lens.aa || lens.radius > 0.0f) rng = ptd::seeded_engine(iter, pix, trace_depth);
    if (lens.aa) {
        fx = fx + (ptd::u01(rng) - 0.5f);
        fy = fy + (ptd::u01(rng) - 0.5f);
    }
    f3 a = ptd::scale(ptd::scale(right, cam.pixelLength[0]), (fx - (float)cam.resolution[0] * 0.5f));
    f3 b = ptd::scale(ptd::scale(up, cam.pixelLength[1]), (fy - (float)cam.resolution[1] * 0.5f));
    ro = pos;
    rd = ptd::normalize(ptd::sub(ptd::sub(view, a), b));
    if (lens.radius > 0.0f) {
        const float ft = lens.focal / ptd::dot(rd, view);
        const f3 focus = ptd::add(pos, ptd::scale(rd, ft));
        const float r = lens.radius * __builtin_sqrtf(ptd::u01(rng));
        const float theta = ptd::u01(rng) * 6.2831853071795864769252867665590057683943f;
        float sa, ca;
        ptd::sincos_shared(theta, sa, ca);
        ro = ptd::add(ptd::add(pos, ptd::scale(right, r * ca)), ptd::scale(up, r * sa));
        rd = ptd::normalize(ptd::sub(focus, ro));
    }
}

}
```

### project3-cuda-path-tracer_amd/csrc/ptmi355.hip

```cpp
#include <hip/hip_runtime.h>

#include <algorithm>
#include <atomic>
#include <cfloat>
#include <cmath>
#include <cstdarg>
#include <cstdio>
#include <cstdlib>
#include <cstring>
#include <type_traits>
#include <vector>

#include "../../include/ptmi355.h"
#include "pt_device.hpp"

static_assert(sizeof(pt_vec3) == 12 && sizeof(pt_mat4) == 64 && sizeof(pt_ray) == 24, "ABI");
static_assert(sizeof(pt_geom) == 236 && offsetof(pt_geom, transform) == 44 &&
              offsetof(pt_geom, inverseTransform) == 108 && offsetof(pt_geom, invTranspose) == 172, "Geom ABI");
static_assert(sizeof(pt_material) == 44 && offsetof(pt_material, hasReflective) == 28 &&
              offsetof(pt_material, emittance) == 40, "Material ABI");
static_assert(sizeof(pt_camera) == 84 && offsetof(pt_camera, view) == 32 &&
              offsetof(pt_camera, pixelLength) == 76, "Camera ABI");
static_assert(sizeof(pt_path_segment) == 44 && offsetof(pt_path_segment, pixelIndex) == 36, "PathSegment ABI");
static_assert(sizeof(pt_shadeable_intersection) == 20 && offsetof(pt_shadeable_intersection, materialId) == 16,
// ... 17 lines not shown
#include "pt_lights.hpp"
#include "pt_kernels.hpp"

#include "pt_h_session.hpp"
#include "pt_h_enqueue.hpp"
#include "pt_h_image.hpp"
#include "pt_h_api.hpp"
#include "pt_h_state.hpp"
#include "pt_h_denoise.hpp"


#include "pt_probe.hpp"
#include "pt_multi.hpp"

extern "C" int ptdbg_counts(unsigned int *out, int words) {
    if (!g_single.live || !g_single.dbg_counts || words < 0 || (size_t)words > g_single.dbg_words) return -1;
    if (hipStreamSynchronize(g_single.stream) != hipSuccess) return -1;
    if (hipMemcpy(out, g_single.dbg_counts, (size_t)words * 4, hipMemcpyDeviceToHost) != hipSuccess) return -1;
    if (hipMemset(g_single.dbg_counts, 0, g_single.dbg_words * 4) != hipSuccess) return -1;
    return words;
}

extern "C" int ptdbg_lookahead(unsigned long long out[4]) {
    if (G.live) {
        for (int k = 0; k < 4; ++k) out[k] = 0;
        for (auto &wp : G.w) {
            const Renderer &c = wp->ctx;
            out[0] += c.la_windows; out[1] += c.la_misses; out[2] += c.la_discards;
        }
        const Renderer &c0 = G.w[0]->ctx;
        out[3] = c0.la[c0.la_cur].valid ? (unsigned long long)c0.la[c0.la_cur].count : 0ull;
        return 0;
    }
    if (!g_single.live) return -1;
    out[0] = g_single.la_windows; out[1] = g_single.la_misses; out[2] = g_single.la_discards;
    out[3] = g_single.la[g_single.la_cur].valid ? (unsigned long long)g_single.la[g_single.la_cur].count : 0ull;
    return 0;
}

extern "C" int ptdbg_lookahead_masked(unsigned long long out[2]) {
    if (G.live) {
        out[0] = 0; out[1] = 0;
        for (auto &wp : G.w) { out[0] += wp->ctx.la_masked_windows; out[1] += wp->ctx.la_masked_calls; }
        return 0;
    }
    if (!g_single.live) return -1;
    out[0] = g_single.la_masked_windows; out[1] = g_single.la_masked_calls;
    return 0;
}

extern "C" int ptdbg_first_hit(unsigned long long out[2]) {
    if (G.live) {
        out[0] = 0; out[1] = 0;
        for (auto &wp : G.w) { out[0] += wp->ctx.first_hit_fills; out[1] += wp->ctx.first_hit_launches; }
        return 0;
    }
    if (!g_single.live) return -1;
    out[0] = g_single.first_hit_fills; out[1] = g_single.first_hit_launches;
    return 0;
}

extern "C" int ptdbg_first_two(unsigned long long out[1]) {
    if (G.live) {
        out[0] = 0;
        for (auto &wp : G.w) out[0] += wp->ctx.first_two_launches;
        return 0;
    }
    if (!g_single.live) return -1;
    out[0] = g_single.first_two_launches;
    return 0;
}

extern "C" int ptdbg_first_state(unsigned long long out[1]) {
    if (G.live) {
        out[0] = 0;
        for (auto &wp : G.w) out[0] += wp->ctx.first_state_launches;
        return 0;
    }
    if (!g_single.live) return -1;
    out[0] = g_single.first_state_launches;
    return 0;
}

extern "C" int ptdbg_denoise(unsigned long long out[3]) {
    if (!g_single.live) return -1;
    for (int k = 0; k < 3; ++k) out[k] = g_single.dn_launches[k];
    return 0;
}

extern "C" int ptdbg_denoise_times(const pt_denoise_params *params, int iter, int reps, float *ms) {
    if (G.live) return fail(PT_ERR_INVALID, "ptdbg_denoise_times: single-device sessions");
    return one::denoise_times(params, iter, reps, ms);
}

extern "C" int ptdbg_temporal(unsigned long long out[2]) {
    if (!g_single.live) return -1;
    for (int k = 0; k < 2; ++k) out[k] = g_single.tp_launches[k];
    return 0;
}

extern "C" int ptdbg_temporal_times(const pt_denoise_params *params, const pt_temporal_params *temporal, int iter, int reps, float *ms) {
    if (G.live) return fail(PT_ERR_INVALID, "ptdbg_temporal_times: single-device sessions");
    return one::temporal_times(params, temporal, iter, reps, ms);
}

extern "C" int ptdbg_variance(unsigned long long out[2]) {
    if (!g_single.live) return -1;
    for (int k = 0; k < 2; ++k) out[k] = g_single.vr_launches[k];
    return 0;
}

extern "C" int ptdbg_variance_times(const pt_variance_params *params, int iter, int reps, float *ms) {
    if (G.live) return fail(PT_ERR_INVALID, "ptdbg_variance_times: single-device sessions");
    return one::variance_times(params, iter, reps, ms);
}

extern "C" int ptdbg_svgf(unsigned long long out[4]) {
    if (!g_single.live) return -1;
    for (int k = 0; k < 4; ++k) out[k] = g_single.sv_launches[k];
    return 0;
}

extern "C" int ptdbg_svgf_times(const pt_variance_params *params, const pt_temporal_params *temporal, int spatial_below, int iter, int reps,
                                float *ms) {
    if (G.live) return fail(PT_ERR_INVALID, "ptdbg_svgf_times: single-device sessions");
    return one::svgf_times(params, temporal, spatial_below, iter, reps, ms);
}

#ifdef PT_WAVE_TIMES
extern "C" int ptdbg_wave_times(unsigned long long *times , uint32_t *hw ) {
    if (hipMemcpyFromSymbol(times, HIP_SYMBOL(g_wave_times), sizeof(unsigned long long) * 8 * 8192 * 2) != hipSuccess) return -1;
    if (hipMemcpyFromSymbol(hw, HIP_SYMBOL(g_wave_hw), sizeof(uint32_t) * 8 * 8192) != hipSuccess) return -1;
    return 0;
}
#endif
```

Baseline: 66370.

## Trace only emitter-aimed rays in the final bounce of plain fused sessions

On the last bounce of a plain fused compacting session, each tile first tests every live ray against the cull boxes of the emissive spheres and cubes. Only rays that could reach an emitter, or that the cull test flags as wild, are packed into the output pool. The normal fused intersect and shade pass then runs on that reduced set, reading from the out pool. This skips intersection and shading for last-bounce paths that cannot gather light, at the cost of an extra culling pass, a pack write and a workgroup fence, plus a new kernel variant that may change occupancy.

```diff
diff --git a/include/ptmi355.h b/include/ptmi355.h
--- a/include/ptmi355.h
+++ b/include/ptmi355.h
@@ -256,6 +256,8 @@
 int pt_probe_tri_form(const pt_triangle *triangles, int count, float origin_bound, const float *origins, const float *directions, int n,
                       uint16_t *ray_slots, int32_t *ray_class, float *form);
 int pt_probe_own_surface_plan(uint64_t paths, int ngeoms, int plain_fused);
+int pt_probe_last_aim_plan(int depth, int trace_depth, int emitters, int ngeoms, int may_fuse, int plain_fused, int plain_shading,
+                           int enabled);
 int pt_num_devices(void);
 const char *pt_exchange_transport(void);
 const char *pt_last_error(void);
diff --git a/profiles/last_aim/count_aimed.py b/profiles/last_aim/count_aimed.py
--- /dev/null
+++ b/profiles/last_aim/count_aimed.py
@@ -0,0 +1,34 @@
+import json
+import os
+import sys
+
+import numpy as np
+
+ROOT = os.path.dirname(os.path.dirname(os.path.dirname(os.path.abspath(__file__))))
+sys.path.insert(0, ROOT)
+sys.path.insert(0, os.path.join(ROOT, "tests"))
+import __graft_entry__ as ge
+from oracle import pyoracle as po
+import last_aim_model as lam
+
+
+def main(path):
+    pt = ge.load_package()
+    scn = pt.load_scene(path)
+    w, h = scn.resolution
+    s = {"geoms": scn.geoms, "materials": scn.materials, "camera": scn.camera, "depth": scn.traceDepth}
+    rays, pix, scored = lam.last_bounce(po, s, 1)
+    mask, _ = lam.aimed(pt, s, rays)
+    tiles, empty = lam.tiles_without(mask)
+    hit = np.isin(pix, scored)
+    em = lam.emitters(scn.geoms, scn.materials)
+    out = {"scene": os.path.relpath(path, ROOT), "frame": [w, h], "depth": scn.traceDepth, "paths": w * h, "primitives": len(scn.geoms),
+           "emitters": em, "form_taken": bool(pt.probe_last_aim_plan(scn.traceDepth - 1, scn.traceDepth, len(em), len(scn.geoms))),
+           "enter_last_bounce": int(len(rays)), "aimed": int(mask.sum()), "aimed_share": float(mask.mean()) if len(rays) else 0.0,
+           "score": int(hit.sum()), "score_outside_the_aimed_set": int((hit & ~mask).sum()),
+           "tiles_of_64": tiles, "tiles_without_an_aimed_lane": empty, "tiles_without_share": (empty / tiles) if tiles else 0.0}
+    print(json.dumps(out, indent=1))
+
+
+if __name__ == "__main__":
+    main(sys.argv[1] if len(sys.argv) > 1 else os.path.join(ROOT, "scenes", "cornell.txt"))
diff --git a/profiles/last_aim/trace_summary.py b/profiles/last_aim/trace_summary.py
--- /dev/null
+++ b/profiles/last_aim/trace_summary.py
@@ -0,0 +1,38 @@
+import csv
+import re
+import statistics as st
+import sys
+from collections import defaultdict
+
+rows = list(csv.DictReader(open(sys.argv[1])))
+by = defaultdict(list)
+for r in rows:
+    by[r["Kernel_Name"]].append((int(r["End_Timestamp"]) - int(r["Start_Timestamp"])) / 1e3)
+print("%8s %10s %10s %10s %10s  name" % ("calls", "median", "mean", "min", "max"))
+for k, v in sorted(by.items(), key=lambda kv: -sum(kv[1])):
+    print("%8d %10.1f %10.1f %10.1f %10.1f  %s" % (len(v), st.median(v), st.mean(v), min(v), max(v), k))
+qkey = "Queue_Id" if "Queue_Id" in rows[0] else None
+skey = "Stream_Id" if "Stream_Id" in rows[0] else qkey
+per = defaultdict(list)
+pos = {}
+for r in sorted(rows, key=lambda r: int(r["Start_Timestamp"])):
+    n = r["Kernel_Name"]
+    if "k_bounce" not in n:
+        continue
+    m = re.search(r"k_bounce<([^>]*)>", n)
+    args = [a.strip() for a in m.group(1).split(",")] if m else []
+    mode = re.sub(r"\(.*?\)", "", args[0]) if args else ""
+    first = len(args) >= 5 and (args[4] in ("true", "1") or mode == "2")
+    two = first and mode in ("3", "4")
+    s = r.get(skey, "0")
+    us = (int(r["End_Timestamp"]) - int(r["Start_Timestamp"])) / 1e3
+    if two:
+        per["0+1"].append(us)
+        pos[s] = 1
+        continue
+    pos[s] = 0 if first else pos.get(s, 0) + 1
+    per[pos[s]].append(us)
+print("\nk_bounce by position in the batch (per %s)" % skey)
+for p in sorted(per, key=lambda p: (0.5 if p == "0+1" else p)):
+    v = per[p]
+    print("bounce%s %s: calls %d median %.1f mean %.1f min %.1f max %.1f" % ("s" if p == "0+1" else "", p, len(v), st.median(v), st.mean(v), min(v), max(v)))
diff --git a/project3-cuda-path-tracer_amd/__init__.py b/project3-cuda-path-tracer_amd/__init__.py
--- a/project3-cuda-path-tracer_amd/__init__.py
+++ b/project3-cuda-path-tracer_amd/__init__.py
@@ -5,7 +5,7 @@
     device_image_ptr, export_intersections, export_paths, get_image, get_stats, intersect_once,
     set_camera, set_lens, synchronize, tonemap, trace_batch, trace_batch_async, trace_begin, trace_bounce,
     trace_end, clear_image, version, has_experiments, set_profiling, get_profile, STAGES, total_rays, counters, cull_boxes, num_devices, exchange_transport, tri_bounds, tri_records,
-    set_image, probe_rng, probe_sincos, probe_sincos_sums, probe_hemisphere, probe_shade_scatter, probe_sqrt, probe_clock, probe_tri_form, probe_own_surface_plan,
+    set_image, probe_rng, probe_sincos, probe_sincos_sums, probe_hemisphere, probe_shade_scatter, probe_sqrt, probe_clock, probe_tri_form, probe_own_surface_plan, probe_last_aim_plan,
     gbuffer, denoise, denoised_device_ptr, DenoiseParams,
     denoise_temporal, history, history_reset, TemporalParams, set_denoise_albedo, albedo,
     set_environment, get_environment, gradient_cubemap, environment_texel, probe_environment,
diff --git a/project3-cuda-path-tracer_amd/binding.py b/project3-cuda-path-tracer_amd/binding.py
--- a/project3-cuda-path-tracer_amd/binding.py
+++ b/project3-cuda-path-tracer_amd/binding.py
@@ -207,6 +207,7 @@
             L.pt_denoise_svgf.argtypes = [C.POINTER(VarianceParams), C.POINTER(TemporalParams), C.c_int, C.c_int, C.c_void_p, C.c_void_p]
             L.pt_svgf_history.argtypes = [C.c_void_p, C.c_void_p, C.c_void_p, C.c_void_p]
             L.pt_svgf_variance.argtypes = [C.c_void_p]
+            L.pt_probe_last_aim_plan.argtypes = [C.c_int] * 8
         except AttributeError:
             if not os.environ.get("PTMI355_LIB"):
                 raise
@@ -960,6 +961,11 @@
     return bool(library().pt_probe_own_surface_plan(int(paths), int(ngeoms), 1 if plain_fused else 0))
 
 
+def probe_last_aim_plan(depth, trace_depth, emitters, ngeoms, may_fuse=True, plain_fused=True, plain_shading=True, enabled=True):
+    return bool(library().pt_probe_last_aim_plan(int(depth), int(trace_depth), int(emitters), int(ngeoms), 1 if may_fuse else 0,
+                                                 1 if plain_fused else 0, 1 if plain_shading else 0, 1 if enabled else 0))
+
+
 def probe_hemisphere(normals, seeds):
     nr = np.ascontiguousarray(normals, dtype=np.float32).reshape(-1, 3)
     sd = np.ascontiguousarray(seeds, dtype=np.uint32)
diff --git a/project3-cuda-path-tracer_amd/csrc/pt_h_api.hpp b/project3-cuda-path-tracer_amd/csrc/pt_h_api.hpp
--- a/project3-cuda-path-tracer_amd/csrc/pt_h_api.hpp
+++ b/project3-cuda-path-tracer_amd/csrc/pt_h_api.hpp
@@ -232,6 +232,9 @@
     if (const char *e = pt_experiment("PTMI355_FIRST_TWO")) R.first_two_enabled = atoi(e) != 0;
     R.first_state_enabled = true;
     if (const char *e = pt_experiment("PTMI355_FIRST_STATE")) R.first_state_enabled = atoi(e) != 0;
+    R.last_aim_enabled = true;
+    if (const char *e = pt_experiment("PTMI355_LAST_AIM")) R.last_aim_enabled = atoi(e) != 0;
+    list_emitters(d);
     R.host_sparse_enabled = (d->flags & (PT_HOST_SPARSE | PT_SHARED_IMAGE)) != 0;
     if (const char *e = pt_experiment("PTMI355_ASYNC_DIRECT")) R.async_direct_enabled = atoi(e) != 0;
     R.pin_enabled = true;
@@ -470,8 +473,9 @@
                                       own ? bounce_fn<MESH_NONE, SHN>(R.scene_lds, true, false, true, true, true) : fns[0]};
             const void *fns_state[2] = {own ? bounce_fn<MESH_NONE, SHN>(R.scene_lds, true, false, false, true, true, true) : fns[0],
                                         own ? bounce_fn<MESH_NONE, SHN>(R.scene_lds, true, false, true, true, true, true) : fns[0]};
+            const void *fns_last[2] = {(own && SH == 0) ? last_aim_fn(R.scene_lds, false) : fns[0], (own && SH == 0) ? last_aim_fn(R.scene_lds, true) : fns[0]};
             for (const void *f : {fns[0], fns[1], fns_own[0], fns_own[1], fns_tab[0], fns_tab[1], fns_tab[2], fns_tab[3], fns_two[0], fns_two[1],
-                                  fns_state[0], fns_state[1]}) {
+                                  fns_state[0], fns_state[1], fns_last[0], fns_last[1]}) {
                 int n = 0;
                 HIPCHK(hipOccupancyMaxActiveBlocksPerMultiprocessor(&n, f, BLOCK, R.lds_bytes));
                 per_cu = std::min(per_cu, n);
diff --git a/project3-cuda-path-tracer_amd/csrc/pt_h_enqueue.hpp b/project3-cuda-path-tracer_amd/csrc/pt_h_enqueue.hpp
--- a/project3-cuda-path-tracer_amd/csrc/pt_h_enqueue.hpp
+++ b/project3-cuda-path-tracer_amd/csrc/pt_h_enqueue.hpp
@@ -143,6 +143,17 @@
     if (slds) return gen ? (const void *)k_bounce<MODE_FUSED, true, MESH, true, true, false, false, SH> : (const void *)k_bounce<MODE_FUSED, true, MESH, true, false, false, false, SH>;
     return gen ? (const void *)k_bounce<MODE_FUSED, true, MESH, false, true, false, false, SH> : (const void *)k_bounce<MODE_FUSED, true, MESH, false, false, false, false, SH>;
 }
+const void *last_aim_fn(bool slds, bool own) {
+    if (own) return slds ? (const void *)k_bounce<MODE_FUSED, true, MESH_NONE, true, false, false, true, 0, true> : (const void *)k_bounce<MODE_FUSED, true, MESH_NONE, false, false, false, true, 0, true>;
+    return slds ? (const void *)k_bounce<MODE_FUSED, true, MESH_NONE, true, false, false, false, 0, true> : (const void *)k_bounce<MODE_FUSED, true, MESH_NONE, false, false, false, false, 0, true>;
+}
+void launch_last_aim(const BounceArgs &a) {
+#define PT_LAST_AIM(SLDS, OWN) \
+    hipLaunchKernelGGL((k_bounce<MODE_FUSED, true, MESH_NONE, SLDS, false, false, OWN, 0, true>), dim3(R.grid), dim3(BLOCK), R.lds_bytes, R.stream, a)
+    if (R.scene_lds) { if (R.own_form) PT_LAST_AIM(true, true); else PT_LAST_AIM(true, false); }
+    else { if (R.own_form) PT_LAST_AIM(false, true); else PT_LAST_AIM(false, false); }
+#undef PT_LAST_AIM
+}
 #define PT_SHADE_DISPATCH_WITH(EXTRA, ...)                                                                  \
     do {                                                                                                    \
         switch ((a.env_n ? SH_ENV : 0) | ((R.flags & PT_GLOSSY) ? SH_GLOSSY : 0)) {                         \
@@ -282,6 +293,11 @@
     R.own_form = own_surface_plan((uint64_t)a.pool_n, R.scene.ngeoms,
                                   compact && !unfused && R.mesh_mode == MESH_NONE && R.sort_keys == 0 &&
                                   R.own_enabled);
+    const bool last_aim = last_aim_plan(depth, R.trace_depth, R.nemit, R.scene.ngeoms, may_fuse && !first2,
+                                        compact && !unfused && !cached0 && R.mesh_mode == MESH_NONE && R.sort_keys == 0,
+                                        a.env_n == 0 && !(R.flags & (PT_GLOSSY | PT_DIRECT_LIGHT | PT_SMOOTH_NORMALS)) &&
+                                            a.tex_tab == nullptr && a.bump_tab == nullptr && a.vnormals == nullptr,
+                                        R.last_aim_enabled);
     if (cached0 && !R.cache_valid) {
         StageTimer tm(PT_STAGE_INTERSECT);
         const Isect cache{R.cache_mem, (uint32_t)R.map.tile_pixels};
@@ -316,6 +332,11 @@
         else if (compact) launch_bounce<MODE_CACHE0, true>(a); else launch_bounce<MODE_CACHE0, false>(a);
     } else if (unfused) {
         if (compact) launch_bounce<MODE_ISECT, true>(a); else launch_bounce<MODE_ISECT, false>(a);
+    } else if (last_aim) {
+        for (int k = 0; k < R.nemit; ++k) a.last_emit[k] = R.emit[k];
+        a.last_nemit = R.nemit;
+        R.last_aim_launches++;
+        launch_last_aim(a);
     } else {
         if (compact) launch_bounce<MODE_FUSED, true>(a); else launch_bounce<MODE_FUSED, false>(a);
     }
diff --git a/project3-cuda-path-tracer_amd/csrc/pt_h_scene.hpp b/project3-cuda-path-tracer_amd/csrc/pt_h_scene.hpp
--- a/project3-cuda-path-tracer_amd/csrc/pt_h_scene.hpp
+++ b/project3-cuda-path-tracer_amd/csrc/pt_h_scene.hpp
@@ -3,6 +3,17 @@
 namespace {
 
 int upload_tri_bounds(const pt_scene_desc *d, double Rorigin);
+
+void list_emitters(const pt_scene_desc *d) {
+    R.nemit = 0;
+    for (int i = 0; i < d->num_geoms; ++i) {
+        const pt_geom &g = d->geoms[i];
+        if (g.type != PT_SPHERE && g.type != PT_CUBE) continue;
+        if (g.materialid < 0 || g.materialid >= d->num_materials || !(d->materials[g.materialid].emittance > 0.0f)) continue;
+        if (R.nemit < LAST_AIM_MAX) R.emit[R.nemit] = i;
+        R.nemit++;
+    }
+}
 
 int upload_cull(const pt_scene_desc *d, const pt_camera &cam) {
     const int n = d->num_geoms;
diff --git a/project3-cuda-path-tracer_amd/csrc/pt_h_session.hpp b/project3-cuda-path-tracer_amd/csrc/pt_h_session.hpp
--- a/project3-cuda-path-tracer_amd/csrc/pt_h_session.hpp
+++ b/project3-cuda-path-tracer_amd/csrc/pt_h_session.hpp
@@ -59,6 +59,10 @@
     uint32_t *state_ended = nullptr;
     bool first_state_enabled = true;
     uint64_t first_state_launches = 0;
+    int emit[LAST_AIM_MAX] = {0, 0, 0, 0};
+    int nemit = 0;
+    bool last_aim_enabled = true;
+    uint64_t last_aim_launches = 0;
     uint64_t first_hit_fills = 0, first_hit_launches = 0;
     Isect isect{};
     float *final_mem = nullptr;
diff --git a/project3-cuda-path-tracer_amd/csrc/pt_k_bounce.hpp b/project3-cuda-path-tracer_amd/csrc/pt_k_bounce.hpp
--- a/project3-cuda-path-tracer_amd/csrc/pt_k_bounce.hpp
+++ b/project3-cuda-path-tracer_amd/csrc/pt_k_bounce.hpp
@@ -31,6 +31,7 @@
     bool kargs = false;
     bool kmisc = false;
     bool epi_direct = false;
+    bool from_out = false;
     SceneAcc acc;
     float *tri_lds;
     int lane, iter0;
@@ -62,7 +63,7 @@
         if (gen_rays) {
             tr.pid = i;
         } else {
-            const SlotPtr p = (c.kargs ? karg_pool(offsetof(BounceArgs, in)) : in).slot(src);
+            const SlotPtr p = (c.kargs ? karg_pool(c.from_out ? offsetof(BounceArgs, out) : offsetof(BounceArgs, in)) : in).slot(src);
             tr.pid = ppid(p);
             ro = ptd::mk(pf(p, 0), pf(p, 1), pf(p, 2));
             rd = ptd::mk(pf(p, 3), pf(p, 4), pf(p, 5));
@@ -435,18 +436,69 @@
     }
 }
 
+template <bool RESOLVE, bool OWN>
+__device__ __forceinline__ void aim_tiles(const BounceArgs &a, const TileCtx &c, int depth, uint32_t first_tile, uint32_t count,
+                                          uint32_t tiles, uint32_t n, bool packed_in, uint32_t span_in, uint32_t &cur,
+                                          uint32_t dst_base, bool aligned, uint32_t &aimed_n, uint32_t &traced) {
+    const int lane = c.lane;
+    for (uint32_t r = 0; r < count; ++r) {
+        const uint32_t tile = first_tile + r;
+        if (tile >= tiles) break;
+        rotate_priority(r + (uint32_t)depth, PT_MIN_WAVES + 1);
+        bool active = false;
+        uint32_t i = 0, src = 0;
+        if (aligned) {
+            const uint32_t *tb = a.dir_in.tbase();
+            while (tile >= tb[cur + 1]) ++cur;
+            const uint32_t t64 = (tile - tb[cur]) * TILE + (uint32_t)lane;
+            active = t64 < a.dir_in.count()[cur];
+            src = cur * span_in + t64;
+            i = a.dir_in.base()[cur] + t64;
+        } else {
+            i = tile * TILE + lane;
+            active = i < n;
+            src = i;
+            if (packed_in) src = resolve_src(a.dir_in, span_in, cur, i, active, a.ctl);
+        }
+        TileRegs tr;
+        f3 ro, rd;
+        uint32_t own;
+        tile_load<false, RESOLVE, OWN>(a, c, a.in, depth, tile, i, src, true, active, tr, ro, rd, own);
+        const CullRay cr = cull_ray(ro, rd, a.scene.rmax);
+        uint64_t m = ballot64(cr.wild);
+        const int ne = karg_field<int>(offsetof(BounceArgs, last_nemit));
+        for (int k = 0; k < ne; ++k) {
+            const int g = karg_field<int>(offsetof(BounceArgs, last_emit) + 4 * (size_t)k);
+            cfloat *cc = as_const(a.scene.cull) + g * CULL_WORDS;
+            m |= ballot64(cull_box(cr, cc[0], cc[1], cc[2], cc[3], cc[4], cc[5]));
+        }
+        const uint64_t act = ballot64(tr.active);
+        m &= act;
+        traced += (uint32_t)__popcll((unsigned long long)act);
+        if (lane_of(m)) {
+            const SlotPtr p = karg_pool(offsetof(BounceArgs, out)).slot(dst_base + aimed_n + rank_below(m));
+            pf(p, 0) = ro.x; pf(p, 1) = ro.y; pf(p, 2) = ro.z;
+            pf(p, 3) = rd.x; pf(p, 4) = rd.y; pf(p, 5) = rd.z;
+            pf(p, 6) = tr.col.x; pf(p, 7) = tr.col.y; pf(p, 8) = tr.col.z;
+            ppid(p) = tr.pid | (OWN ? own << OWN_SHIFT : 0u);
+        }
+        aimed_n += (uint32_t)__popcll((unsigned long long)m);
+    }
+}
+
 #ifdef PT_WAVE_TIMES
 __device__ unsigned long long g_wave_times[8][8192][2];
 __device__ uint32_t g_wave_hw[8][8192];
 #endif
 
-template <int MODE, bool COMPACT, int MESH, bool SLDS, bool GEN = false, bool SORT = false, bool OWN = false, int SH = 0>
+template <int MODE, bool COMPACT, int MESH, bool SLDS, bool GEN = false, bool SORT = false, bool OWN = false, int SH = 0, bool LAST = false>
 __global__ __launch_bounds__(BLOCK, MESH == MESH_TILES ? PT_LOOP_WAVES : (MESH == MESH_PRE && PT_PRE_WAVES > PT_MIN_WAVES) ? PT_PRE_WAVES : (SORT && MODE == MODE_FUSED && MESH == MESH_NONE) ? PT_SORT_WAVES : ((MODE == MODE_FUSED || MODE == MODE_CACHE0 || mode_first2(MODE)) && COMPACT && MESH == MESH_NONE && !SORT && PT_FUSED_WAVES > PT_MIN_WAVES) ? PT_FUSED_WAVES : PT_MIN_WAVES) void k_bounce(BounceArgs a) {
     static_assert(!OWN || ((MODE == MODE_FUSED || MODE == MODE_CACHE0 || mode_first2(MODE)) && COMPACT && MESH == MESH_NONE && !SORT),
                   "own-surface form: the plain fused compacting kernel, or the table form of its bounce 0");
     static_assert(!mode_first2(MODE) || (COMPACT && MESH == MESH_NONE && GEN && !SORT), "MODE_FIRST2 / MODE_STATE2: the plain compacting pipeline's first launch");
     static_assert(MODE != MODE_STATE2 || SH == 0, "MODE_STATE2: sessions without environment map or lobes");
     static_assert((SH & SH_SMOOTH) == 0 || (MODE == MODE_FUSED && MESH != MESH_NONE), "the SMOOTH forms: the fused kernel of a session with a mesh");
+    static_assert(!LAST || (MODE == MODE_FUSED && COMPACT && MESH == MESH_NONE && !GEN && !SORT && SH == 0), "the aimed last bounce: the plain fused compacting kernel");
 #ifdef PT_WAVE_TIMES
     const unsigned long long wt0 = __builtin_amdgcn_s_memrealtime();
 #endif
@@ -493,6 +545,20 @@
         if (packed_in && wid * R < tiles)
             cur = aligned ? find_range(a.dir_in.tbase(), a.dir_in.nr, wid * R) : find_range(a.dir_in.base(), a.dir_in.nr, wid * R * TILE);
         STAMP(2);
+        if constexpr (LAST) {
+            uint32_t aimed_n = 0;
+            aim_tiles<RESOLVE, OWN>(a, c, a.depth, wid * R, R, tiles, n, packed_in, span_in, cur, wid * R * TILE, aligned, aimed_n, traced);
+            __builtin_amdgcn_fence(__ATOMIC_ACQ_REL, "workgroup");
+            asm volatile("s_waitcnt vmcnt(0) lgkmcnt(0)" ::: "memory");
+            TileCtx c2 = c;
+            c2.from_out = true;
+            WgSpans ws{};
+            ws.p1 = ws.p2 = ws.p3 = 0xffffffffu; ws.total = aimed_n;
+            ws.b0 = ws.b1 = ws.b2 = ws.b3 = wid * R * TILE;
+            uint32_t traced2 = 0;
+            run_tiles<MODE, COMPACT, MESH, false, false, DEFER, false, OWN, SH>(a, c2, q, a.out, a.out, a.depth, 0, (aimed_n + TILE - 1) / TILE, tiles, n,
+                                                      false, 0, cur, wid * R * TILE, true, ws, packed, traced2);
+        } else
         run_tiles<MODE, COMPACT, MESH, GEN, SORT, DEFER, RESOLVE, OWN, SH>(a, c, q, a.in, a.out, a.depth, wid * R, R, tiles, n, packed_in, span_in,
                                                   cur, wid * R * TILE, false, WgSpans{}, packed, traced, W * R * TILE, aligned);
         if (COMPACT) {
diff --git a/project3-cuda-path-tracer_amd/csrc/pt_probe.hpp b/project3-cuda-path-tracer_amd/csrc/pt_probe.hpp
--- a/project3-cuda-path-tracer_amd/csrc/pt_probe.hpp
+++ b/project3-cuda-path-tracer_amd/csrc/pt_probe.hpp
@@ -556,6 +556,10 @@
     return own_surface_plan(paths, ngeoms, plain_fused != 0) ? 1 : 0;
 }
 
+int pt_probe_last_aim_plan(int depth, int trace_depth, int emitters, int ngeoms, int may_fuse, int plain_fused, int plain_shading, int enabled) {
+    return last_aim_plan(depth, trace_depth, emitters, ngeoms, may_fuse != 0, plain_fused != 0, plain_shading != 0, enabled != 0) ? 1 : 0;
+}
+
 int pt_probe_hemisphere(const float *normals, const uint32_t *seeds, int n, float *dirs) {
     if (n < 0 || (n > 0 && (!normals || !seeds || !dirs))) return fail(PT_ERR_INVALID, "pt_probe_hemisphere: bad argument");
     if (n == 0) return PT_OK;
diff --git a/project3-cuda-path-tracer_amd/csrc/pt_types.hpp b/project3-cuda-path-tracer_amd/csrc/pt_types.hpp
--- a/project3-cuda-path-tracer_amd/csrc/pt_types.hpp
+++ b/project3-cuda-path-tracer_amd/csrc/pt_types.hpp
@@ -39,6 +39,12 @@
 constexpr uint64_t OWN_MAX_PATHS = 1ull << OWN_SHIFT;
 inline bool own_surface_plan(uint64_t paths, int ngeoms, bool plain_fused) {
     return plain_fused && ngeoms >= 1 && ngeoms <= OWN_MAX_GEOMS && paths <= OWN_MAX_PATHS;
+}
+constexpr int LAST_AIM_MAX = 4;
+inline bool last_aim_plan(int depth, int trace_depth, int nemit, int ngeoms, bool may_fuse, bool plain_fused, bool plain_shading,
+                          bool enabled) {
+    return enabled && may_fuse && plain_fused && plain_shading && trace_depth >= 3 && depth == trace_depth - 1 &&
+           nemit >= 0 && nemit <= LAST_AIM_MAX && 2 * nemit < ngeoms;
 }
 
 template <typename T>
@@ -249,6 +255,8 @@
     const uint32_t *first_ended;
     uint32_t first_ended_tiles;
     const float *vnormals;
+    int last_emit[LAST_AIM_MAX];
+    int last_nemit;
 };
 
 enum : uint32_t { FS_ZERO = 0, FS_CONST = 1, FS_DIFFUSE = 2, FS_FIXED = 3, FS_KIND_MASK = 3 };
diff --git a/project3-cuda-path-tracer_amd/csrc/ptmi355.hip b/project3-cuda-path-tracer_amd/csrc/ptmi355.hip
--- a/project3-cuda-path-tracer_amd/csrc/ptmi355.hip
+++ b/project3-cuda-path-tracer_amd/csrc/ptmi355.hip
@@ -123,6 +123,17 @@
     return 0;
 }
 
+extern "C" int ptdbg_last_aim(unsigned long long out[1]) {
+    if (G.live) {
+        out[0] = 0;
+        for (auto &wp : G.w) out[0] += wp->ctx.last_aim_launches;
+        return 0;
+    }
+    if (!g_single.live) return -1;
+    out[0] = g_single.last_aim_launches;
+    return 0;
+}
+
 extern "C" int ptdbg_denoise(unsigned long long out[3]) {
     if (!g_single.live) return -1;
     for (int k = 0; k < 3; ++k) out[k] = g_single.dn_launches[k];
```

Result: slower. 65380 (-1.5%).
